# akashsengupta1997/STRAPS-3DHumanShapePose

Measured on AMD Instinct MI355X. Metric: bodies/sec, higher is better.
Workload: dtype fp32 (encoder convolutions as exact bf16x3 operand splits (six bf16 products per term); in-step SMPL blend contraction and skinning as 3-product fp16 splits (fp16x3_lbs: 22-bit operands); fp32 accumulate throughout)

## Files before the change

include/straps_hip.h:

```cpp
#ifndef STRAPS_HIP_H
#define STRAPS_HIP_H

#include <stddef.h>
#include <stdint.h>

#ifdef __cplusplus
extern "C" {
#endif

#define STRAPS_ABI_VERSION 12

#define STRAPS_OK 0
#define STRAPS_EINVAL 1
#define STRAPS_EHIP 2
#define STRAPS_EUNSUPPORTED 3

int straps_abi_version(void);
int straps_selftest_mfma_peak(const float* seed512, float* out, int blocks, int iters, void* stream);
int straps_selftest_mfma_bf16(float* out, unsigned long long* clk2, int blocks, int iters, void* stream);
int straps_selftest_mfma_bf16_dense(float* out, unsigned long long* clk2, int blocks, int iters, int data, void* stream);
const char* straps_last_error(void);
int straps_device_count(void);
int straps_wall_clock_khz(void);
int straps_set_clock_accumulator(unsigned long long* acc2);
// ... 221 lines not shown
                          unsigned short* draw_planes, long long plane_stride, void* workspace, long long rows, int c,
                          int accumulate, void* stream);
int straps_bn_bwd_finish_bits_x3(const float* dy, const unsigned* relu_bits, const float* raw, const float* save_mean,
                                 const float* save_invstd, const float* gamma, float* dgamma, float* dbeta, float* draw,
                                 unsigned short* draw_planes, long long plane_stride, const double* partials, int nblk,
                                 void* workspace, long long rows, int c, int accumulate, void* stream);
int straps_conv_dgrad_x3_bits(const unsigned short* dy3, long long dy_plane_stride, const unsigned short* w3_crsk,
                              long long w_plane_stride, const float* addend, float* dx_nhwc, int batch, int h, int w,
                              int cin, int cout, int kh, int kw, int stride, int pad, int tile_cfg,
                              const unsigned* addend_bits, void* stream);
int straps_conv_dgrad_x3_bn_bits(const unsigned short* dy3, long long dy_plane_stride,
                                 const unsigned short* w3_crsk, long long w_plane_stride, const float* addend,
                                 float* dx_nhwc, int batch, int h, int w, int cin, int cout, int kh, int kw,
                                 int stride, int pad, int tile_cfg, const float* bn_raw, const float* bn_out,
                                 const float* bn_mask_scale, const float* bn_mask_shift, const float* bn_mean,
                                 const float* bn_invstd, double* bn_partials, const unsigned* addend_bits,
                                 const unsigned* bn_out_bits, void* stream);
int straps_conv_wgrad_x3_on_planes(int batch, int h, int w, int cin, int cout, int kh, int kw,
                                   int stride, int pad);
int straps_conv_wgrad_x3(const float* x_nhwc, const float* dy_nhwc, const unsigned short* x3,
                         long long x_plane_stride, const unsigned short* dy3, long long dy_plane_stride,
                         float* dw_oihw, void* workspace, int batch, int h, int w, int cin, int cout,
                         int kh, int kw, int stride, int pad, int accumulate, void* stream);


size_t straps_conv_wgrad_workspace_bytes(int batch, int h, int w, int cin, int cout, int kh,
                                         int kw, int stride, int pad);
int straps_conv_wgrad(const float* x_nhwc, const float* dy_nhwc, float* dw_oihw, void* workspace,
                      int batch, int h, int w, int cin, int cout, int kh, int kw, int stride,
                      int pad, int accumulate, void* stream);
#define STRAPS_WG_ROUTE_F32 0
#define STRAPS_WG_ROUTE_PLANES 1
#define STRAPS_WG_ROUTE_F32_1X1 2
#define STRAPS_WG_FAMILY_TAP_F32 0
#define STRAPS_WG_FAMILY_HALO_F32 1
#define STRAPS_WG_FAMILY_TAP_X3 2
#define STRAPS_WG_FAMILY_HALO_X3 3
#define STRAPS_WG_FAMILY_TAP_X3F 4
typedef struct straps_wgrad_plan_t {
    int32_t family;
    int32_t bco, bci;
    int32_t chunk_px;
    int32_t tiles;
    int32_t splits;
    int32_t unit;
    int32_t units;
    int32_t taps;
    int32_t lds_bytes;
    int64_t part_bytes;
} straps_wgrad_plan_t;
int straps_conv_wgrad_plan(int route, int batch, int h, int w, int cin, int cout, int kh, int kw, int stride, int pad,
                           straps_wgrad_plan_t* out);
size_t straps_stem_wgrad_workspace_bytes(int batch, int cin, int h, int w);
int straps_stem_wgrad(const float* x_nchw, const float* dy_nhwc, float* dw_oihw, void* workspace,
                      const uint32_t* nzmask , int batch, int cin,
                      int h, int w, int accumulate, void* stream);
#define STRAPS_STEM_DGRAD_MAX_CIN 64
size_t straps_stem_dgrad_weight_floats(int cin);
int straps_pack_stem_dgrad_weight(const float* w_oihw, float* w_pk, int cin, void* stream);
int straps_stem_dgrad(const float* dy_nhwc, const float* w_pk, float* dx_nchw, int batch, int cin, int h, int w,
                      int accumulate, void* stream);
int straps_bn_bwd_blocks(long long rows, int c);
size_t straps_bn_bwd_workspace_bytes(long long rows, int c);
int straps_bn_bwd(const float* dy, const float* yact, const float* raw, const float* save_mean,
                  const float* save_invstd, const float* gamma, const float* mask_scale,
                  const float* mask_shift, float* dgamma, float* dbeta, float* draw, float* dz_out,
                  void* workspace, long long rows, int c, int accumulate, void* stream);
int straps_bn_relu_maxpool_fwd(const float* raw_nhwc, const float* scale, const float* shift,
                               float* y_pool_nhwc, uint8_t* idx, int batch, int h, int w, int c,
                               void* stream);
int straps_bn_bwd_pooled(const float* dy_pool_nhwc, const uint8_t* idx, const float* raw,
                         const float* save_mean, const float* save_invstd, const float* gamma,
                         const float* mask_scale, const float* mask_shift, float* dgamma, float* dbeta,
                         float* draw, void* workspace, int batch, int h, int w, int c, int accumulate,
                         void* stream);
size_t straps_stem_tiles(int batch, int in_h, int in_w);
int straps_stem_tile_activity(const uint32_t* nzmask, uint8_t* tile_active, int batch, int cin, int in_h,
                              int in_w, void* stream);
int straps_bn_bwd_pooled_sparse(const float* dy_pool_nhwc, const uint8_t* idx, const float* raw,
                                const float* save_mean, const float* save_invstd, const float* gamma,
                                const float* mask_scale, const float* mask_shift, float* dgamma,
                                float* dbeta, float* draw, void* workspace, int batch, int h, int w, int c,
                                int accumulate, const uint8_t* tile_active, void* stream);
int straps_maxpool_fwd_idx(const float* x_nhwc, float* y_nhwc, uint8_t* idx, int batch, int h,
                           int w, int c, void* stream);
int straps_maxpool_bwd(const float* dy_nhwc, const uint8_t* idx, float* dx_nhwc, int batch, int h,
                       int w, int c, void* stream);
int straps_gap_bwd(const float* dfeat, float* dx_nhwc, int batch, int hw, int c, void* stream);
int straps_masked_copy(const float* x, int ldx, const float* mask, int ldmask, float* y, int ldy,
                       int m, int n, int accumulate, void* stream);
int straps_rot6d_bwd(const float* x6, long long ld, int per_row, const float* drot, float* dx6,
                     long long ldd, long long rows, void* stream);

int straps_build_proxy_input(const float* seg, const float* joints2d, float* out_nchw, int batch,
                             int nj, int wh, void* stream);
int straps_build_proxy_input_std(const float* seg, const float* joints2d, float* out_nchw, int batch,
                                 int nj, int wh, int std, void* stream);
int straps_build_proxy_input_nz(const float* seg, const float* joints2d, float* out_nchw, uint32_t* nzmask,
                                int batch, int nj, int wh, int std, void* stream);
size_t straps_loss_workspace_bytes(long long batch);
int straps_loss_fwd_bwd(const float* pred_verts, const float* pred_joints, const float* est,
                        int ld_est, const float* pred_rot, const float* tgt_verts,
                        const float* tgt_joints2d, const float* tgt_joints3d,
                        const float* tgt_shape, const float* tgt_rot, const float* log_vars,
                        float* loss_out, float* dverts, float* djoints, float* dest, float* drot,
                        float* dlogvar, void* workspace, long long batch, int img_wh, void* stream);
int straps_loss_fwd_bwd_gm(const float* pred_verts, const float* pred_joints, const float* est, int ld_est,
                           const float* pred_rot, const float* tgt_verts, const float* tgt_joints2d,
                           const float* tgt_joints3d, const float* tgt_shape, const float* tgt_rot,
                           const float* log_vars, float* loss_out, float* dverts, float* djoints, float* dest,
                           float* drot, float* dlogvar, void* workspace, long long batch, int img_wh,
                           const float* j2d_count_global, float count_scale, void* stream);
int straps_count_visible(const float* tgt_joints2d, float* out_count, long long batch, int nj, int img_wh,
                         void* stream);
int straps_mse_fwd(const float* pred, const float* tgt, const uint8_t* row_mask, long long rows,
                   int cols, float tgt_scale, float tgt_shift, float* out3, void* workspace,
                   void* stream);
int straps_mse_bwd(const float* pred, const float* tgt, const uint8_t* row_mask, long long rows,
                   int cols, float tgt_scale, float tgt_shift, const float* coef, float* grad,
                   void* stream);
int straps_augment_seg(const float* seg, const float* uniforms, const float* remove_prob,
                       float occlude_prob, int box_dim, float* out, int batch, int wh, void* stream);
int straps_philox_fill(unsigned long long seed, const long long* step_dev, long long step_host,
                       unsigned substream, float* out, long long n, int kind, void* stream);
int straps_counter_add(long long* counters, int n, long long delta, void* stream);
int straps_gather_f32(const float* src, const int* index, float* dst, int n, void* stream);
int straps_memset_zero(void* ptr, size_t bytes, void* stream);
int straps_augment_smpl(const float* pose_rows, long long n_rows, const float* u_index,
                        const float* orig_shape, const float* mean_shape, const float* shape_draws,
                        int shape_mode, const float* std_vector, double range_lo, double range_hi,
                        float* out_shape, float* out_rotmats, float* out_pose, long long batch,
                        void* stream);
int straps_augment_cam_t(const float* mean_cam_t, const float* normals_xy, const float* uniform_z,
                         double xy_std, double z_lo, double z_hi, float* out_cam_t, long long batch,
                         void* stream);
int straps_deviate_joints2d(const float* joints2d, const float* uniforms, double lo, double hi,
                            double hip_lo, double hip_hi, float* out, long long batch, void* stream);
int straps_deviate_verts2d(const float* verts, const float* uniforms, double lo, double hi, float* out,
                           long long nverts_total, void* stream);
int straps_project_targets(const float* joints, const float* cam_t, float fx, float fy, float cx,
                           float cy, float* joints2d, float* joints3d, long long batch, void* stream);
size_t straps_rasterize_workspace_bytes(long long batch, int nverts, int wh);
int straps_rasterize_parts(const float* verts, const int32_t* faces, const uint8_t* face_parts,
                           const float* cam_K, const float* cam_R, const float* cam_t, float* parts,
                           float* depth, void* workspace, long long batch, int nverts, int nfaces, int wh,
                           int cam_per_body, float near, float far, const float* vert_noise_u, double noise_lo,
                           double noise_hi, void* stream);
int straps_crop_resize(const float* seg, const float* joints2d, const float* uniforms,
                       double orig_scale_factor, double delta_scale_lo, double delta_scale_hi,
                       double delta_centre_lo, double delta_centre_hi, float* out_seg,
                       float* out_joints2d, int* boxes, int batch, int wh, int out_wh, int nj,
                       void* stream);
int straps_predict_proxy_input(const uint8_t* sil, const float* joints2d, int ld_joint,
                               const float* gauss_patch, int std, double bbox_scale_factor,
                               float* out_nchw, float* out_joints2d, int32_t* boxes,
                               int batch, int h, int w, int nj, int out_wh, void* stream);
int straps_point_metrics(const float* pred, const float* target, float* out3, long long batch,
                         int npoints, void* stream);
int straps_point_align(const float* pred, const float* target, float* out3, float* pred_sc,
                       float* pred_pa, long long batch, int npoints, void* stream);
int straps_silhouette_counts(const uint8_t* pred, const uint8_t* target, int32_t* counts4,
                             long long batch, long long npix, void* stream);
size_t straps_wp_silhouette_workspace_bytes(long long batch, int nverts);
int straps_wp_silhouette(const float* verts, const int32_t* faces, const float* cam_wp, uint8_t* mask,
                         void* workspace, long long batch, int nverts, int nfaces, int wh, void* stream);
int straps_adam_step(float* params, const float* grads, float* exp_avg, float* exp_avg_sq,
// ... 105 lines not shown
```

straps-3dhumanshapepose_amd/autograd_ops.py:

```python
import ctypes as C

import torch

from . import hipabi
from .encoder_exec import encoder_forward
from .ief_module import EST_LD


def _empty_like(t):
    return torch.empty_like(t, memory_format=torch.contiguous_format)


class GradSink(dict):

    def __init__(self, views=None):
        super().__init__()
        self.views = views

    def buf(self, p, zero=False):
        if self.views is not None and p in self.views:
            return self.views[p]
        return torch.zeros_like(p) if zero else torch.empty_like(p)


# ... 156 lines not shown
                                                   k, k, stride, pad, 0, hipabi.ptr(bn_next['raw']), hipabi.ptr(None if from_raw else bn_next['out']),
                                                   hipabi.ptr(ssn[0] if from_raw else None), hipabi.ptr(ssn[1] if from_raw else None),
                                                   hipabi.ptr(ssn[2]), hipabi.ptr(ssn[3]), hipabi.ptr(part), hipabi.stream_ptr()),
                         'straps_conv_dgrad_x3_bn')
            bn_next['bwd_partials'] = (part, nblk, dx)
            return dx
        if addend_bits is not None:
            hipabi.check(L.straps_conv_dgrad_x3_bits(hipabi.ptr(g3), gps, hipabi.ptr(w3), wps, hipabi.ptr(addend), hipabi.ptr(dx), B, H, W, Cin, Cout,
                                                     k, k, stride, pad, 0, hipabi.ptr(addend_bits), hipabi.stream_ptr()), 'straps_conv_dgrad_x3_bits')
            return dx
        hipabi.check(L.straps_conv_dgrad_x3(hipabi.ptr(g3), gps, hipabi.ptr(w3), wps, hipabi.ptr(addend), hipabi.ptr(dx), B, H, W, Cin, Cout,
                                            k, k, stride, pad, 0, hipabi.stream_ptr()), 'straps_conv_dgrad_x3')
        return dx
    if addend_bits is not None:
        raise RuntimeError('ReLU bits exist only on the bf16x3 route')
    hipabi.check(L.straps_conv_dgrad(hipabi.ptr(draw), hipabi.ptr(_packed_dgrad_weight(net, conv)), hipabi.ptr(addend), hipabi.ptr(dx), B, H, W,
                                     Cin, Cout, k, k, stride, pad, 0, hipabi.stream_ptr()), 'straps_conv_dgrad')
    return dx


def encoder_backward(net, tape, dfeat, views=None, side_stream=None, after_layer3=None, want_dx=False, param_grads=True):
    L = hipabi.lib()
    grads = GradSink(views)
    side = _SideStream(side_stream)
    sink = {} if getattr(net, 'conv_precision', 'fp32') == 'bf16x3' else None

    def sink_of(rec):
        return None if rec.get('fmode') else sink

    def keep(rec):
        if sink is None or rec.get('x3') is None:
            return True
        B, H, W, Cin, Cout, k, stride, pad, Ho, Wo = rec['geom']
        return not L.straps_conv_wgrad_x3_on_planes(B, H, W, Cin, Cout, k, k, stride, pad)
    rec = tape['gap']
    B, HW, Cf = rec['geom']
    dy = _empty_like(rec['x'])
    hipabi.check(L.straps_gap_bwd(hipabi.ptr(dfeat.contiguous()), hipabi.ptr(dy), B, HW, Cf, hipabi.stream_ptr()), 'straps_gap_bwd')
    units = [u for li in range(1, 5) for u in getattr(net, 'layer%d' % li)]
    for li in range(4, 0, -1):
        for unit in reversed(list(getattr(net, 'layer%d' % li))):
            pairs = unit.conv_bn_pairs()
            ui = units.index(unit)
            prev_last = tape[id(units[ui - 1].conv_bn_pairs()[-1][0])] if ui > 0 else None
            rec = tape[id(pairs[-1][0])]
            ubits = rec.get('bits') if sink is not None else None
            dskip_bits = None
            if ubits is not None:
                draw, _ = _bn_bwd(L, rec, dy, True, False, grads, sink_of(rec), keep(rec))
                dz = dy
            else:
                draw, dz = _bn_bwd(L, rec, dy, True, True, grads, sink_of(rec), keep(rec))
            if param_grads:
                side.run(lambda rec=rec, draw=draw: _conv_wgrad(L, rec, draw, grads, sink), draw)
            if unit.downsample is not None:
                recd = tape[id(unit.downsample[0])]
                drawd, _ = _bn_bwd(L, recd, dz, False, False, grads, sink_of(recd), keep(recd), mask_bits=ubits)
                if param_grads:
                    side.run(lambda recd=recd, drawd=drawd: _conv_wgrad(L, recd, drawd, grads, sink), drawd)
                dskip = _conv_dgrad(L, net, recd, drawd, None, sink)
            else:
                dskip, dskip_bits = dz, ubits
            for ci in range(len(pairs) - 1, 0, -1):
                rec_prev = tape[id(pairs[ci - 1][0])]
                dt = _conv_dgrad(L, net, tape[id(pairs[ci][0])], draw, None, sink, bn_next=rec_prev if sink is not None else None)
                rec = rec_prev
                draw, _ = _bn_bwd(L, rec, dt, True, False, grads, sink_of(rec), keep(rec))
                if param_grads:
                    side.run(lambda rec=rec, draw=draw: _conv_wgrad(L, rec, draw, grads, sink), draw)
            dy = _conv_dgrad(L, net, tape[id(pairs[0][0])], draw, dskip, sink, bn_next=prev_last if sink is not None else None,
                             addend_bits=dskip_bits)
        if li == 3 and after_layer3 is not None:
            side.join()
            after_layer3()
    rec = tape['maxpool']
    B, H, W, Cc, Hp, Wp = rec['geom']
    if rec['kind'] == 'maxpool_fused':
        idx = rec['idx']
        rec = tape['stem']
        bn, raw, ss = rec['bn'], rec['raw'], rec['stats']
        ws = torch.empty(L.straps_bn_bwd_workspace_bytes(B * H * W, Cc) // 4, device=raw.device, dtype=torch.float32)
        dgamma, dbeta = grads.buf(bn.weight), grads.buf(bn.bias)
        draw = _empty_like(raw)
        tact = None
        if rec.get('nzmask') is not None and _SPARSE_STEM_TAIL and not want_dx:
            _, Cin0, Hin, Win = rec['geom'][:4]
            tact = torch.empty(L.straps_stem_tiles(B, Hin, Win), device=raw.device, dtype=torch.uint8)
            hipabi.check(L.straps_stem_tile_activity(hipabi.ptr(rec['nzmask']), hipabi.ptr(tact), B, Cin0, Hin, Win, hipabi.stream_ptr()),
                         'straps_stem_tile_activity')
        hipabi.check(L.straps_bn_bwd_pooled_sparse(hipabi.ptr(dy), hipabi.ptr(idx), hipabi.ptr(raw), hipabi.ptr(ss[2]), hipabi.ptr(ss[3]),
                                                   hipabi.ptr(bn.weight), hipabi.ptr(ss[0]), hipabi.ptr(ss[1]), hipabi.ptr(dgamma), hipabi.ptr(dbeta),
                                                   hipabi.ptr(draw), hipabi.ptr(ws), B, H, W, Cc, 2 if rec.get('frozen') else 0, hipabi.ptr(tact),
                                                   hipabi.stream_ptr()), 'straps_bn_bwd_pooled_sparse')
        grads[bn.weight] = dgamma
        grads[bn.bias] = dbeta
    else:
        dstem = _empty_like(rec['x'])
        hipabi.check(L.straps_maxpool_bwd(hipabi.ptr(dy), hipabi.ptr(rec['idx']), hipabi.ptr(dstem), B, H, W, Cc, hipabi.stream_ptr()),
                     'straps_maxpool_bwd')
        rec = tape['stem']
        draw, _ = _bn_bwd(L, rec, dstem, True, False, grads)
    B, Cin, H, W, Ho, Wo = rec['geom']
    dx = None
    if want_dx:
        dx = torch.empty(B, Cin, H, W, device=draw.device, dtype=torch.float32)
        hipabi.check(L.straps_stem_dgrad(hipabi.ptr(draw), hipabi.ptr(net._packed_stem_dgrad_weight()), hipabi.ptr(dx), B, Cin, H, W, 0,
                                         hipabi.stream_ptr()), 'straps_stem_dgrad')
    if param_grads:
        ws = torch.empty(L.straps_stem_wgrad_workspace_bytes(B, Cin, H, W) // 4, device=draw.device, dtype=torch.float32)
        dw = grads.buf(net.conv1.weight)
        hipabi.check(L.straps_stem_wgrad(hipabi.ptr(rec['x']), hipabi.ptr(draw), hipabi.ptr(dw), hipabi.ptr(ws), hipabi.ptr(rec.get('nzmask')),
                                         B, Cin, H, W, 0, hipabi.stream_ptr()), 'straps_stem_wgrad')
        grads[net.conv1.weight] = dw
    side.join()
    return (grads, dx) if want_dx else grads


def ief_backward(ief, feat, tape, dest, views=None, param_grads=True):
    sink = GradSink(views)
    L, st = hipabi.lib(), hipabi.stream_ptr()
    pk = ief._packed(feat.device)
    B, F = feat.shape
    H1, H2, P = ief.fc1.out_features, ief.fc2.out_features, ief.num_output_params
    dev = feat.device
    T = len(tape)
    e = lambda *s: torch.empty(*s, device=dev, dtype=torch.float32)
    D = hipabi.gemm_desc
    ests, h1s, h2s = tape[0]['stacks']
    assert ests.shape == (T + 1, B, EST_LD) and h1s.shape == (T, B, H1) and h2s.shape == (T, B, H2)
    dW3, db3 = sink.buf(ief.fc3.weight), sink.buf(ief.fc3.bias)
    dW2, db2 = sink.buf(ief.fc2.weight), sink.buf(ief.fc2.bias)
    dW1, db1 = sink.buf(ief.fc1.weight), sink.buf(ief.fc1.bias)
    dests = e(T + 1, B, EST_LD)
    dsrc = dest if dest.stride(-1) == 1 and dest.dim() == 2 else dest.contiguous()
    hipabi.check(L.straps_masked_copy(hipabi.ptr(dsrc), dsrc.stride(0), None, 0, hipabi.ptr(dests[T]), EST_LD, B, EST_LD, 0, st), 'ief dest slot')
    dh2s, dh1s, dc1 = e(T, B, H2), e(T, B, H1), e(B, H1)
    w3, w2 = ief.fc3.weight, ief.fc2.weight
    for it in reversed(range(T)):
        hipabi.gemm_multi([D(dests[it + 1], EST_LD, 1, w3, H2, 1, dh2s[it], H2, B, H2, P, mask=h2s[it], ldmask=H2)])
        hipabi.gemm_multi([D(dh2s[it], H2, 1, w2, H1, 1, dh1s[it], H1, B, H1, H2, mask=h1s[it], ldmask=H1,
                             c2=dc1, ldc2=H1, accumulate2=int(it != T - 1))])
        hipabi.gemm_multi([D(dh1s[it], H1, 1, pk['w1e'], EST_LD, 1, dests[it], EST_LD, B, P, H1, addend=dests[it + 1], ldadd=EST_LD)])
    one = pk['one']
    dfeat = e(B, F)
    if not param_grads:
        hipabi.gemm_multi([D(dc1, H1, 1, pk['w1f'], F, 1, dfeat, F, B, F, H1)])
        return dfeat, {}
    KB = T * B
    hipabi.gemm_multi([
        D(dh2s, 1, H2, h1s, H1, 1, dW2, H1, H2, H1, KB),
        D(dc1, 1, H1, feat, F, 1, dW1, F + P, H1, F, B),
        D(dh1s, 1, H1, ests, EST_LD, 1, dW1.data_ptr() + 4 * F, F + P, H1, P, KB),
        D(dests[1], 1, EST_LD, h2s, H2, 1, dW3, H2, P, H2, KB),
        D(dc1, H1, 1, pk['w1f'], F, 1, dfeat, F, B, F, H1),
        D(one, 0, 0, dh2s, H2, 1, db2, H2, 1, H2, KB),
        D(one, 0, 0, dests[1], EST_LD, 1, db3, P, 1, P, KB),
        D(one, 0, 0, dc1, H1, 1, db1, H1, 1, H1, B)])
    grads = {ief.fc1.weight: dW1, ief.fc1.bias: db1, ief.fc2.weight: dW2, ief.fc2.bias: db2, ief.fc3.weight: dW3, ief.fc3.bias: db3}
    return dfeat, grads


class _RegressorFn(torch.autograd.Function):

    @staticmethod
    def forward(ctx, reg, x, *params):
        enc_tape, ief_tape = {}, []
        with torch.no_grad():
            feat = encoder_forward(reg.image_encoder, x, enc_tape)
            est = reg.ief_module.forward_estimate(feat, ief_tape)
        ctx.reg, ctx.feat, ctx.enc_tape, ctx.ief_tape, ctx.params = reg, feat, enc_tape, ief_tape, params
        return est

# ... 171 lines not shown
```

straps-3dhumanshapepose_amd/csrc/backward.hip:

```cpp
#include "common.h"
#include <stdlib.h>

namespace {


constexpr int TY = 2, TX = 32, PH = 2 * TY + 5, PW = 72, TPIX = TY * TX;
constexpr int CG = 4, GK = CG * 49, GNB = (GK + 31) / 32, GUNITS = 2 * GNB, UPW = (GUNITS + 3) / 4;

__global__ __launch_bounds__(256) void stem_tileact_kernel(const unsigned* __restrict__ nzmask, uint8_t* __restrict__ tact, int C, int H, int W,
                                                           int tiles_x, int tiles_y, int ntiles, int groups) {
    const int idx = blockIdx.x * 256 + threadIdx.x;
    if (idx >= ntiles * groups) return;
    const int grp = idx / ntiles, tile = idx - grp * ntiles;
    int bid = tile;
    const int b = bid / (tiles_x * tiles_y);
    bid -= b * tiles_x * tiles_y;
    const int ty = bid / tiles_x, tx = bid - ty * tiles_x;
    const int hi0 = 2 * (ty * TY) - 3, wi0 = 2 * (tx * TX) - 3;
    const int HC = (H + 3) >> 2, WW = (W + 255) >> 8;
    const int rc0 = max(hi0, 0) >> 2, rc1 = min(hi0 + PH - 1, H - 1) >> 2;
    const int wa = max(wi0 - 1, 0), wb = min(wi0 - 2 + PW, W - 1);
    const int c0 = grp * CG, nc = min(CG, C - c0);
    unsigned chact = 0;
    for (int cl = 0; cl < nc; ++cl) {
// ... 343 lines not shown
        double t[8];
#pragma unroll
        for (int e = 0; e < 8; ++e) t[e] = red[tc][e];
        for (int q = 1; q < TR; ++q)
#pragma unroll
            for (int e = 0; e < 8; ++e) t[e] += red[q * 16 + tc][e];
        double* o = part + ((long long)blockIdx.x * C + c4 * 4) * 2;
#pragma unroll
        for (int e = 0; e < 4; ++e) { o[e * 2 + 0] = t[e]; o[e * 2 + 1] = t[4 + e]; }
    }
}

__global__ __launch_bounds__(256) void bn_bwd_reduce_pooled_kernel(const float* __restrict__ raw, const float* __restrict__ mean,
                                                                   const float* __restrict__ invstd, const float* __restrict__ msc,
                                                                   const float* __restrict__ msh, double* __restrict__ part, long long prows,
                                                                   int C, int rows_per_block, PoolSrc ps) {
    __shared__ double red[256][8];
    constexpr int TR = 16;
    const int tc = threadIdx.x & 15, tr = threadIdx.x >> 4;
    const int c4 = blockIdx.y * 16 + tc;
    const bool active = c4 * 4 < C;
    const long long r0 = (long long)blockIdx.x * rows_per_block;
    const long long r1 = r0 + rows_per_block < prows ? r0 + rows_per_block : prows;
    double s1[4] = {0.0, 0.0, 0.0, 0.0}, s2[4] = {0.0, 0.0, 0.0, 0.0};
    f32x4 is = {0.f, 0.f, 0.f, 0.f};
    if (active) {
        const f32x4 mu = *reinterpret_cast<const f32x4*>(mean + c4 * 4);
        is = *reinterpret_cast<const f32x4*>(invstd + c4 * 4);
        const f32x4 ksc = *reinterpret_cast<const f32x4*>(msc + c4 * 4), ksh = *reinterpret_cast<const f32x4*>(msh + c4 * 4);
        for (long long r = r0 + tr; r < r1; r += TR) {
            const int wo = (int)(r % ps.Wo);
            const long long t = r / ps.Wo;
            const int ho = (int)(t % ps.Ho);
            const long long b = t / ps.Ho;
            const long long o = r * C + c4 * 4;
            const f32x4 d = *reinterpret_cast<const f32x4*>(ps.dyp + o);
            const uchar4 k4 = *reinterpret_cast<const uchar4*>(ps.idx + o);
            const int k[4] = {k4.x, k4.y, k4.z, k4.w};
            float xr[4];
#pragma unroll
            for (int e = 0; e < 4; ++e) {
                const int hi = 2 * ho - 1 + k[e] / 3, wi = 2 * wo - 1 + k[e] % 3;
                xr[e] = raw[((b * ps.H + hi) * ps.W + wi) * C + c4 * 4 + e];
            }
#pragma unroll
            for (int e = 0; e < 4; ++e) {
                const float g = fmaf(xr[e], ksc[e], ksh[e]) > 0.f ? d[e] : 0.f;
                s1[e] += (double)g;
                s2[e] += (double)g * ((double)xr[e] - (double)mu[e]);
            }
        }
    }
#pragma unroll
    for (int e = 0; e < 4; ++e) { red[threadIdx.x][e] = s1[e]; red[threadIdx.x][4 + e] = s2[e] * (double)is[e]; }
    __syncthreads();
    if (tr == 0 && active) {
        double t[8];
#pragma unroll
        for (int e = 0; e < 8; ++e) t[e] = red[tc][e];
        for (int q = 1; q < TR; ++q)
#pragma unroll
            for (int e = 0; e < 8; ++e) t[e] += red[q * 16 + tc][e];
        double* o = part + ((long long)blockIdx.x * C + c4 * 4) * 2;
#pragma unroll
        for (int e = 0; e < 4; ++e) { o[e * 2 + 0] = t[e]; o[e * 2 + 1] = t[4 + e]; }
    }
}

__global__ __launch_bounds__(256) void bn_bwd_finalize_kernel(const double* __restrict__ part, int nblocks, int C, double count,
                                                             const float* __restrict__ gamma, const float* __restrict__ invstd,
                                                             float* __restrict__ dgamma, float* __restrict__ dbeta,
                                                             double* __restrict__ coefd, float* __restrict__ k1, int accumulate) {
    int c;
    double s1, s2;
    if (bn_partials_sum4(part, nblocks, C, s1, s2, c)) {
        dbeta[c] = accumulate ? dbeta[c] + (float)s1 : (float)s1;
        dgamma[c] = accumulate ? dgamma[c] + (float)s2 : (float)s2;
        k1[c] = gamma[c] * invstd[c];
        coefd[c] = s1 / count;
        coefd[C + c] = s2 / count;
    }
}

constexpr int POOL_CHUNK = 1024;
template <bool POOL>
__global__ __launch_bounds__(256) void bn_bwd_apply_kernel(const float* __restrict__ dy, const float* __restrict__ yact,
                                                           const float* __restrict__ raw, const float* __restrict__ mean,
                                                           const float* __restrict__ invstd, const double* __restrict__ coefd,
                                                           const float* __restrict__ k1p, const float* __restrict__ msc,
                                                           const float* __restrict__ msh, float* __restrict__ draw, float* dz_out,
                                                           u16* __restrict__ planes, long long pstride, long long n4, int C, PoolSrc ps,
                                                           const unsigned* __restrict__ bits, int tiled) {
    const int C4 = C >> 2;
    const long long first = POOL ? (long long)blockIdx.x * POOL_CHUNK + threadIdx.x : (long long)blockIdx.x * 256 + threadIdx.x;
    const long long last = POOL ? (n4 < ((long long)blockIdx.x + 1) * POOL_CHUNK ? n4 : ((long long)blockIdx.x + 1) * POOL_CHUNK) : n4;
    const long long step = POOL ? 256 : (long long)gridDim.x * 256;
    const long long rows = n4 / C4;
    struct Consts { f32x4 ksc, ksh, mu, is, k1; double m1[4], m2[4]; };
    auto load_consts = [&](int c4) {
        Consts k;
        if (!yact && !bits && msc) { k.ksc = *reinterpret_cast<const f32x4*>(msc + c4 * 4); k.ksh = *reinterpret_cast<const f32x4*>(msh + c4 * 4); }
        k.mu = *reinterpret_cast<const f32x4*>(mean + c4 * 4);
        k.is = *reinterpret_cast<const f32x4*>(invstd + c4 * 4);
        k.k1 = *reinterpret_cast<const f32x4*>(k1p + c4 * 4);
#pragma unroll
        for (int e = 0; e < 4; ++e) { k.m1[e] = coefd[c4 * 4 + e]; k.m2[e] = coefd[C + c4 * 4 + e]; }
        return k;
    };
    auto body = [&](long long idx, long long row, int c4, const Consts& k) {
        f32x4 g;
        if constexpr (POOL) {
            if (ps.tany) {
                const int wi = (int)(row % ps.W);
                const long long t = row / ps.W;
                const int hi = (int)(t % ps.H);
                const long long b = t / ps.H;
                if (!ps.tany[(b * ps.tiles_y + (hi >> 1)) * ps.tiles_x + (wi >> 5)]) return;
            }
            g = pool_grad(ps, row, c4, C);
        } else {
            g = *reinterpret_cast<const f32x4*>(dy + idx * 4);
        }
        const f32x4 xr = *reinterpret_cast<const f32x4*>(raw + idx * 4);
        if (bits) {
            const unsigned nib = bits[row * (C >> 5) + (c4 >> 3)] >> ((c4 & 7) * 4);
#pragma unroll
            for (int e = 0; e < 4; ++e) g[e] = ((nib >> e) & 1u) ? g[e] : 0.f;
        } else if (yact) {
            const f32x4 ya = *reinterpret_cast<const f32x4*>(yact + idx * 4);
#pragma unroll
            for (int e = 0; e < 4; ++e) g[e] = ya[e] > 0.f ? g[e] : 0.f;
        } else if (msc) {
#pragma unroll
            for (int e = 0; e < 4; ++e) g[e] = fmaf(xr[e], k.ksc[e], k.ksh[e]) > 0.f ? g[e] : 0.f;
        }
        f32x4 o;
#pragma unroll
        for (int e = 0; e < 4; ++e) {
            const double xh = ((double)xr[e] - (double)k.mu[e]) * (double)k.is[e];
            o[e] = (float)((double)k.k1[e] * (((double)g[e] - k.m1[e]) - xh * k.m2[e]));
        }
        if (dz_out) *reinterpret_cast<f32x4*>(dz_out + idx * 4) = g;
        if (draw) *reinterpret_cast<f32x4*>(draw + idx * 4) = o;
        if (planes) store_planes4_cm(planes, pstride, row, c4 * 4, rows, o);
    };
    if (!POOL && tiled) {
        const int l = threadIdx.x & 63, w = threadIdx.x >> 6, wcg = tiled, ncb = (C4 >> 4) / wcg, trows = 16 / wcg;
        const int c4 = ((int)(blockIdx.x % ncb) * wcg + w % wcg) * 16 + (l >> 5) * 8 + (l & 7);
        const Consts k = load_consts(c4);
        const long long rstep = (long long)(gridDim.x / ncb) * trows;
        for (long long row = (long long)(blockIdx.x / ncb) * trows + (w / wcg) * 4 + ((l >> 3) & 3); row < rows; row += rstep) body(row * C4 + c4, row, c4, k);
    } else if (step % C4 == 0) {
        if (first >= last) return;
        const int c4 = (int)(first % C4);
        const Consts k = load_consts(c4);
        const long long rstep = step / C4;
        long long row = first / C4;
        for (long long idx = first; idx < last; idx += step, row += rstep) body(idx, row, c4, k);
    } else {
        for (long long idx = first; idx < last; idx += step) {
            const int c4 = (int)(idx % C4);
            body(idx, idx / C4, c4, load_consts(c4));
        }
    }
}

__global__ __launch_bounds__(256) void maxpool_idx_kernel(const float* __restrict__ x, float* __restrict__ y, uint8_t* __restrict__ idx,
                                                          int B, int H, int W, int C, int Ho, int Wo) {
    const int C4 = C >> 2;
    const long long n = (long long)B * Ho * Wo * C4;
    for (long long i = (long long)blockIdx.x * 256 + threadIdx.x; i < n; i += (long long)gridDim.x * 256) {
        const int c4 = (int)(i % C4);
        long long t = i / C4;
        const int wo = (int)(t % Wo); t /= Wo;
        const int ho = (int)(t % Ho);
        const int b = (int)(t / Ho);
        f32x4 m = {-INFINITY, -INFINITY, -INFINITY, -INFINITY};
        int am[4] = {0, 0, 0, 0};
        bool first = true;
#pragma unroll
        for (int r = 0; r < 3; ++r) {
            const int hi = 2 * ho - 1 + r;
            if ((unsigned)hi >= (unsigned)H) continue;
#pragma unroll
            for (int s = 0; s < 3; ++s) {
                const int wi = 2 * wo - 1 + s;
                if ((unsigned)wi >= (unsigned)W) continue;
                const f32x4 v = *reinterpret_cast<const f32x4*>(x + (((long long)b * H + hi) * W + wi) * C + c4 * 4);
#pragma unroll
                for (int e = 0; e < 4; ++e)
                    if (first || v[e] > m[e] || v[e] != v[e]) { m[e] = v[e]; am[e] = r * 3 + s; }
                first = false;
            }
        }
        *reinterpret_cast<f32x4*>(y + i * 4) = m;
        *reinterpret_cast<uchar4*>(idx + i * 4) = make_uchar4((unsigned char)am[0], (unsigned char)am[1], (unsigned char)am[2], (unsigned char)am[3]);
    }
}

__global__ __launch_bounds__(256) void bn_relu_maxpool_kernel(const float* __restrict__ raw, const float* __restrict__ scale,
                                                              const float* __restrict__ shift, float* __restrict__ y, uint8_t* __restrict__ idx,
                                                              u16* __restrict__ planes, long long pstride, int B, int H, int W, int C, int Ho, int Wo) {
    const int C4 = C >> 2;
    const long long n = (long long)B * Ho * Wo * C4;
    for (long long i = (long long)blockIdx.x * 256 + threadIdx.x; i < n; i += (long long)gridDim.x * 256) {
        const int c4 = (int)(i % C4);
        long long t = i / C4;
        const int wo = (int)(t % Wo); t /= Wo;
        const int ho = (int)(t % Ho);
        const int b = (int)(t / Ho);
        const f32x4 sc = *reinterpret_cast<const f32x4*>(scale + c4 * 4);
        const f32x4 sh = *reinterpret_cast<const f32x4*>(shift + c4 * 4);
        f32x4 m = {-INFINITY, -INFINITY, -INFINITY, -INFINITY};
        int am[4] = {0, 0, 0, 0};
        bool first = true;
#pragma unroll
        for (int r = 0; r < 3; ++r) {
            const int hi = 2 * ho - 1 + r;
            if ((unsigned)hi >= (unsigned)H) continue;
#pragma unroll
            for (int s = 0; s < 3; ++s) {
                const int wi = 2 * wo - 1 + s;
                if ((unsigned)wi >= (unsigned)W) continue;
                f32x4 v = *reinterpret_cast<const f32x4*>(raw + (((long long)b * H + hi) * W + wi) * C + c4 * 4);
#pragma unroll
                for (int e = 0; e < 4; ++e) {
                    v[e] = fmaxf(fmaf(v[e], sc[e], sh[e]), 0.f);
                    if (first || v[e] > m[e] || v[e] != v[e]) { m[e] = v[e]; am[e] = r * 3 + s; }
                }
                first = false;
            }
        }
        *reinterpret_cast<f32x4*>(y + i * 4) = m;
        *reinterpret_cast<uchar4*>(idx + i * 4) = make_uchar4((unsigned char)am[0], (unsigned char)am[1], (unsigned char)am[2], (unsigned char)am[3]);
        if (planes) store_planes4_cm(planes, pstride, i / C4, c4 * 4, (long long)B * Ho * Wo, m);
    }
}

__global__ __launch_bounds__(256) void maxpool_bwd_kernel(const float* __restrict__ dy, const uint8_t* __restrict__ idx,
                                                          float* __restrict__ dx, int B, int H, int W, int C, int Ho, int Wo) {
    const int C4 = C >> 2;
    const long long n = (long long)B * H * W * C4;
    for (long long i = (long long)blockIdx.x * 256 + threadIdx.x; i < n; i += (long long)gridDim.x * 256) {
        const int c4 = (int)(i % C4);
        long long t = i / C4;
        const int wi = (int)(t % W); t /= W;
        const int hi = (int)(t % H);
        const int b = (int)(t / H);
        f32x4 g = {0.f, 0.f, 0.f, 0.f};
        const int ho_lo = hi >> 1, ho_hi = (hi + 1) >> 1;
        const int wo_lo = wi >> 1, wo_hi = (wi + 1) >> 1;
        for (int ho = ho_lo; ho <= ho_hi; ++ho) {
            if (ho >= Ho) continue;
            const int r = hi - (2 * ho - 1);
            for (int wo = wo_lo; wo <= wo_hi; ++wo) {
                if (wo >= Wo) continue;
                const int s = wi - (2 * wo - 1);
                const long long o = (((long long)b * Ho + ho) * Wo + wo) * C + c4 * 4;
                const uchar4 k = *reinterpret_cast<const uchar4*>(idx + o);
                const f32x4 d = *reinterpret_cast<const f32x4*>(dy + o);
                const int want = r * 3 + s;
                if (k.x == want) g[0] += d[0];
                if (k.y == want) g[1] += d[1];
                if (k.z == want) g[2] += d[2];
                if (k.w == want) g[3] += d[3];
            }
        }
        *reinterpret_cast<f32x4*>(dx + i * 4) = g;
    }
}

__global__ __launch_bounds__(256) void gap_bwd_kernel(const float* __restrict__ dfeat, float* __restrict__ dx, int B, int HW, int C) {
    const long long n = (long long)B * HW * C;
    const float inv = 1.0f / (float)HW;
    for (long long i = (long long)blockIdx.x * 256 + threadIdx.x; i < n; i += (long long)gridDim.x * 256) {
        const int c = (int)(i % C);
        const long long b = i / ((long long)HW * C);
        dx[i] = dfeat[b * C + c] * inv;
    }
}

__global__ __launch_bounds__(256) void masked_copy_kernel(const float* __restrict__ x, int ldx, const float* __restrict__ mask, int ldm,
                                                          float* y, int ldy, int M, int N, int accumulate) {
    const long long i = (long long)blockIdx.x * 256 + threadIdx.x;
    if (i >= (long long)M * N) return;
    const int m = (int)(i / N), n = (int)(i - (long long)m * N);
    float v = x[(long long)m * ldx + n];
    if (mask) v = mask[(long long)m * ldm + n] > 0.f ? v : 0.f;
    float* o = y + (long long)m * ldy + n;
    *o = accumulate ? *o + v : v;
}

__global__ __launch_bounds__(256) void rot6d_bwd_kernel(const float* __restrict__ x6, long long ld, int per_row,
                                                        const float* __restrict__ dR, float* __restrict__ dx6, long long ldd,
                                                        long long n) {
    const long long idx = (long long)blockIdx.x * 256 + threadIdx.x;
    if (idx >= n) return;
    const long long row = idx / per_row;
    const int j = (int)(idx - row * per_row);
    const float* x = x6 + row * ld + j * 6;
    const float a1[3] = {x[0], x[2], x[4]}, a2[3] = {x[1], x[3], x[5]};
    const float* g = dR + idx * 9;
    float gb1[3] = {g[0], g[3], g[6]}, gb2[3] = {g[1], g[4], g[7]};
    const float gb3[3] = {g[2], g[5], g[8]};
    const float n1r = sqrtf(a1[0] * a1[0] + a1[1] * a1[1] + a1[2] * a1[2]);
    const float n1 = fmaxf(n1r, 1e-12f);
    const float b1[3] = {a1[0] / n1, a1[1] / n1, a1[2] / n1};
    const float d = b1[0] * a2[0] + b1[1] * a2[1] + b1[2] * a2[2];
    const float u[3] = {a2[0] - d * b1[0], a2[1] - d * b1[1], a2[2] - d * b1[2]};
    const float n2r = sqrtf(u[0] * u[0] + u[1] * u[1] + u[2] * u[2]);
    const float n2 = fmaxf(n2r, 1e-12f);
    const float b2[3] = {u[0] / n2, u[1] / n2, u[2] / n2};
    gb1[0] += b2[1] * gb3[2] - b2[2] * gb3[1];
    gb1[1] += b2[2] * gb3[0] - b2[0] * gb3[2];
    gb1[2] += b2[0] * gb3[1] - b2[1] * gb3[0];
    gb2[0] += gb3[1] * b1[2] - gb3[2] * b1[1];
    gb2[1] += gb3[2] * b1[0] - gb3[0] * b1[2];
    gb2[2] += gb3[0] * b1[1] - gb3[1] * b1[0];
// ... 31 lines not shown
}

}

static int stem_wgrad_blocks(int ntiles) {
    static const int cap = STRAPS_TOOL_ENV_INT("STRAPS_STEM_WGRAD_BLOCKS", 256);
    return ntiles < cap ? ntiles : cap;
}

extern "C" size_t straps_stem_wgrad_workspace_bytes(int batch, int cin, int h, int w) {
    const int Ho = (h - 1) / 2 + 1, Wo = (w - 1) / 2 + 1;
    const int ntiles = batch * ((Ho + TY - 1) / TY) * ((Wo + TX - 1) / TX);
    const int Kp = (cin * 49 + 31) / 32 * 32;
    const size_t groups = (cin + CG - 1) / CG;
    return (size_t)stem_wgrad_blocks(ntiles) * 64 * Kp * sizeof(float) + straps_stem_nzmask_words(batch, cin, h, w) * sizeof(uint32_t) +
           ((groups * ntiles + 3) & ~(size_t)3);
}

extern "C" int straps_stem_wgrad(const float* x_nchw, const float* dy_nhwc, float* dw_oihw, void* workspace, const uint32_t* nzmask,
                                 int batch, int cin, int h, int w, int accumulate, void* stream) {
    STRAPS_REQUIRE(x_nchw && dy_nhwc && dw_oihw && workspace, "straps_stem_wgrad: null pointer");
    STRAPS_REQUIRE(batch > 0 && cin > 0 && h >= 7 && w >= 7, "straps_stem_wgrad: bad shape B=%d C=%d H=%d W=%d", batch, cin, h, w);
    const int K = cin * 49, Kp = (K + 31) / 32 * 32;
    const int Ho = (h - 1) / 2 + 1, Wo = (w - 1) / 2 + 1;
    const int tiles_x = (Wo + TX - 1) / TX, tiles_y = (Ho + TY - 1) / TY;
    const int ntiles = batch * tiles_x * tiles_y;
    const int nblk = stem_wgrad_blocks(ntiles);
    const int groups = (cin + CG - 1) / CG;
    STRAPS_REQUIRE(groups <= 65535, "straps_stem_wgrad: too many input channels (%d)", cin);
    hipStream_t st = (hipStream_t)stream;
    float* part = (float*)workspace;
    uint32_t* own = (uint32_t*)(part + (size_t)nblk * 64 * Kp);
    uint8_t* tact = (uint8_t*)(own + straps_stem_nzmask_words(batch, cin, h, w));
    if (!nzmask) {
        const int rc = straps_stem_nzmask(x_nchw, own, batch, cin, h, w, stream);
        if (rc != STRAPS_OK) return rc;
        nzmask = own;
    }
    hipLaunchKernelGGL(stem_tileact_kernel, dim3((ntiles * groups + 255) / 256), dim3(256), 0, st, nzmask, tact, cin, h, w, tiles_x, tiles_y, ntiles,
                       groups);
    STRAPS_CHECK_LAUNCH("stem_tileact_kernel");
    static const int rot = STRAPS_TOOL_ENV_INT("STRAPS_STEM_WGRAD_ROT", 97);
    hipLaunchKernelGGL(stem_wgrad_kernel, dim3(nblk, groups), dim3(256), 0, st, x_nchw, dy_nhwc, part, tact, batch, cin, h, w, Ho, Wo,
                       tiles_x, tiles_y, Kp, ntiles, rot);
    STRAPS_CHECK_LAUNCH("stem_wgrad_kernel");
    hipLaunchKernelGGL(stem_wgrad_reduce_kernel, dim3((64 * K + 63) / 64), dim3(256), 0, st, (const float*)workspace, dw_oihw, nblk, K, Kp, accumulate);
    STRAPS_CHECK_LAUNCH("stem_wgrad_reduce_kernel");
    return STRAPS_OK;
}

static double bn_bwd_count(long long rows, int flags) { return (flags & 2) ? (double)INFINITY : (double)rows; }

extern "C" int straps_bn_bwd_blocks(long long rows, int c) {
    const int colblocks = (c + 63) / 64;
    long long b = 2048 / colblocks;
    const long long cap = (rows + 63) / 64;
    if (b > cap) b = cap;
    return (int)(b < 1 ? 1 : b);
}

static int bn_bwd_x3_impl(const float* dy, const float* yact, const unsigned* relu_bits, const float* raw, const float* save_mean, const float* save_invstd,
                          const float* gamma, const float* mask_scale, const float* mask_shift, float* dgamma, float* dbeta, float* draw,
                          float* dz_out, unsigned short* draw_planes, long long plane_stride, void* workspace, long long rows, int c,
                          int accumulate, void* stream) {
    STRAPS_REQUIRE(!relu_bits || (!yact && (c & 31) == 0), "straps_bn_bwd_bits_x3: the bits replace yact (and need c %% 32 == 0; c=%d)", c);
    STRAPS_REQUIRE(!draw_planes || (plane_stride >= rows * c && plane_stride % 8 == 0), "straps_bn_bwd_x3: plane_stride must be >= rows*c and a multiple of 8");
    STRAPS_REQUIRE(!draw_planes || (c & 31) == 0, "straps_bn_bwd_x3: chunk-major planes need c %% 32 == 0 (c=%d)", c);
    STRAPS_REQUIRE(dy && raw && save_mean && save_invstd && gamma && dgamma && dbeta && (draw || draw_planes) && workspace, "straps_bn_bwd: null pointer");
    STRAPS_REQUIRE(rows > 0 && c > 0 && (c & 3) == 0, "straps_bn_bwd: bad shape rows=%lld c=%d", rows, c);
    const int C4 = c >> 2;
    STRAPS_REQUIRE(C4 <= 256 ? (256 % C4 == 0) : (C4 % 256 == 0), "straps_bn_bwd: channel count %d not supported", c);
    hipStream_t st = (hipStream_t)stream;
    const int nblk = straps_bn_bwd_blocks(rows, c);
    const int rpb = (int)((rows + nblk - 1) / nblk);
    double* part = (double*)workspace;
    double* coefd = part + (size_t)nblk * c * 2;
    float* k1 = (float*)(coefd + 2 * (size_t)c);
    hipLaunchKernelGGL(bn_bwd_reduce_kernel<false>, dim3(nblk, (c + 63) / 64), dim3(256), 0, st, dy, yact, raw, save_mean, save_invstd, mask_scale, mask_shift, part, rows, c, rpb, PoolSrc{}, relu_bits);
    STRAPS_CHECK_LAUNCH("bn_bwd_reduce_kernel");
    hipLaunchKernelGGL(bn_bwd_finalize_kernel, dim3((c + 3) / 4), dim3(256), 0, st, part, nblk, c, bn_bwd_count(rows, accumulate), gamma, save_invstd, dgamma, dbeta, coefd, k1, accumulate & 1);
    STRAPS_CHECK_LAUNCH("bn_bwd_finalize_kernel");
    const long long n4 = rows * C4;
    const int tiled = straps_bn_tiled(rows, c >> 2);
    hipLaunchKernelGGL(bn_bwd_apply_kernel<false>, dim3(tiled ? straps_bn_tiled_grid(rows, c >> 2, tiled) : straps_grid256_rows(n4, c >> 2)), dim3(256), 0, st, dy, yact, raw, save_mean, save_invstd, coefd, k1, mask_scale, mask_shift, draw, dz_out, draw_planes, plane_stride, n4, c, PoolSrc{}, relu_bits, tiled);
    STRAPS_CHECK_LAUNCH("bn_bwd_apply_kernel");
    return STRAPS_OK;
}

extern "C" int straps_bn_bwd_x3(const float* dy, const float* yact, const float* raw, const float* save_mean, const float* save_invstd,
                                const float* gamma, const float* mask_scale, const float* mask_shift, float* dgamma, float* dbeta, float* draw,
                                float* dz_out, unsigned short* draw_planes, long long plane_stride, void* workspace, long long rows, int c,
                                int accumulate, void* stream) {
    return bn_bwd_x3_impl(dy, yact, nullptr, raw, save_mean, save_invstd, gamma, mask_scale, mask_shift, dgamma, dbeta, draw, dz_out, draw_planes,
                          plane_stride, workspace, rows, c, accumulate, stream);
}

extern "C" int straps_bn_bwd_bits_x3(const float* dy, const unsigned* relu_bits, const float* raw, const float* save_mean, const float* save_invstd,
                                     const float* gamma, float* dgamma, float* dbeta, float* draw, unsigned short* draw_planes, long long plane_stride,
                                     void* workspace, long long rows, int c, int accumulate, void* stream) {
    STRAPS_REQUIRE(relu_bits, "straps_bn_bwd_bits_x3: null bit mask");
    return bn_bwd_x3_impl(dy, nullptr, relu_bits, raw, save_mean, save_invstd, gamma, nullptr, nullptr, dgamma, dbeta, draw, nullptr, draw_planes,
                          plane_stride, workspace, rows, c, accumulate, stream);
}

static int bn_bwd_finish_x3_impl(const float* dy, const float* yact, const unsigned* relu_bits, const float* raw, const float* save_mean,
                                 const float* save_invstd, const float* gamma, const float* mask_scale, const float* mask_shift, float* dgamma,
                                 float* dbeta, float* draw, float* dz_out, unsigned short* draw_planes, long long plane_stride, const double* partials,
                                 int nblk, void* workspace, long long rows, int c, int accumulate, void* stream) {
    STRAPS_REQUIRE(!relu_bits || (!yact && (c & 31) == 0), "straps_bn_bwd_finish_bits_x3: the bits replace yact (and need c %% 32 == 0; c=%d)", c);
    STRAPS_REQUIRE(!draw_planes || (plane_stride >= rows * c && plane_stride % 8 == 0), "straps_bn_bwd_finish_x3: plane_stride must be >= rows*c and a multiple of 8");
    STRAPS_REQUIRE(!draw_planes || (c & 31) == 0, "straps_bn_bwd_finish_x3: chunk-major planes need c %% 32 == 0 (c=%d)", c);
    STRAPS_REQUIRE(dy && raw && save_mean && save_invstd && gamma && dgamma && dbeta && (draw || draw_planes) && workspace && partials && nblk > 0,
                   "straps_bn_bwd_finish_x3: null pointer");
    STRAPS_REQUIRE(rows > 0 && c > 0 && (c & 3) == 0, "straps_bn_bwd_finish_x3: bad shape rows=%lld c=%d", rows, c);
    const int C4 = c >> 2;
    STRAPS_REQUIRE(C4 <= 256 ? (256 % C4 == 0) : (C4 % 256 == 0), "straps_bn_bwd_finish_x3: channel count %d not supported", c);
    hipStream_t st = (hipStream_t)stream;
    double* coefd = (double*)workspace;
    float* k1 = (float*)(coefd + 2 * (size_t)c);
    hipLaunchKernelGGL(bn_bwd_finalize_kernel, dim3((c + 3) / 4), dim3(256), 0, st, partials, nblk, c, bn_bwd_count(rows, accumulate), gamma, save_invstd, dgamma, dbeta, coefd, k1, accumulate & 1);
    STRAPS_CHECK_LAUNCH("bn_bwd_finalize_kernel");
    const long long n4 = rows * C4;
    const int tiled = straps_bn_tiled(rows, c >> 2);
    hipLaunchKernelGGL(bn_bwd_apply_kernel<false>, dim3(tiled ? straps_bn_tiled_grid(rows, c >> 2, tiled) : straps_grid256_rows(n4, c >> 2)), dim3(256), 0, st, dy, yact, raw, save_mean, save_invstd, coefd, k1, mask_scale, mask_shift, draw, dz_out, draw_planes, plane_stride, n4, c, PoolSrc{}, relu_bits, tiled);
    STRAPS_CHECK_LAUNCH("bn_bwd_apply_kernel");
    return STRAPS_OK;
}

extern "C" int straps_bn_bwd_finish_x3(const float* dy, const float* yact, const float* raw, const float* save_mean, const float* save_invstd,
                                       const float* gamma, const float* mask_scale, const float* mask_shift, float* dgamma, float* dbeta,
                                       float* draw, float* dz_out, unsigned short* draw_planes, long long plane_stride, const double* partials,
                                       int nblk, void* workspace, long long rows, int c, int accumulate, void* stream) {
    return bn_bwd_finish_x3_impl(dy, yact, nullptr, raw, save_mean, save_invstd, gamma, mask_scale, mask_shift, dgamma, dbeta, draw, dz_out, draw_planes,
                                 plane_stride, partials, nblk, workspace, rows, c, accumulate, stream);
}

extern "C" int straps_bn_bwd_finish_bits_x3(const float* dy, const unsigned* relu_bits, const float* raw, const float* save_mean,
                                            const float* save_invstd, const float* gamma, float* dgamma, float* dbeta, float* draw,
                                            unsigned short* draw_planes, long long plane_stride, const double* partials, int nblk, void* workspace,
                                            long long rows, int c, int accumulate, void* stream) {
    STRAPS_REQUIRE(relu_bits, "straps_bn_bwd_finish_bits_x3: null bit mask");
    return bn_bwd_finish_x3_impl(dy, nullptr, relu_bits, raw, save_mean, save_invstd, gamma, nullptr, nullptr, dgamma, dbeta, draw, nullptr, draw_planes,
                                 plane_stride, partials, nblk, workspace, rows, c, accumulate, stream);
}

extern "C" int straps_bn_bwd(const float* dy, const float* yact, const float* raw, const float* save_mean, const float* save_invstd,
                             const float* gamma, const float* mask_scale, const float* mask_shift, float* dgamma, float* dbeta, float* draw,
                             float* dz_out, void* workspace, long long rows, int c, int accumulate, void* stream) {
    return straps_bn_bwd_x3(dy, yact, raw, save_mean, save_invstd, gamma, mask_scale, mask_shift, dgamma, dbeta, draw, dz_out, nullptr, 0, workspace,
                            rows, c, accumulate, stream);
}

extern "C" size_t straps_stem_tiles(int batch, int h, int w) {
    const int Ho = (h - 1) / 2 + 1, Wo = (w - 1) / 2 + 1;
    return (size_t)batch * ((Wo + TX - 1) / TX) * ((Ho + TY - 1) / TY);
}

extern "C" int straps_stem_tile_activity(const uint32_t* nzmask, uint8_t* tile_active, int batch, int cin, int h, int w, void* stream) {
    STRAPS_REQUIRE(nzmask && tile_active, "straps_stem_tile_activity: null pointer");
    STRAPS_REQUIRE(batch > 0 && cin > 0 && h >= 7 && w >= 7, "straps_stem_tile_activity: bad shape B=%d C=%d H=%d W=%d", batch, cin, h, w);
    const int Ho = (h - 1) / 2 + 1, Wo = (w - 1) / 2 + 1;
    const int tiles_x = (Wo + TX - 1) / TX, tiles_y = (Ho + TY - 1) / TY;
    const int ntiles = batch * tiles_x * tiles_y;
    hipLaunchKernelGGL(stem_tileany_kernel, dim3((unsigned)(((long long)ntiles * 32 + 255) / 256)), dim3(256), 0, (hipStream_t)stream, nzmask, tile_active, cin, h, w, tiles_x, tiles_y,
                       ntiles);
    STRAPS_CHECK_LAUNCH("stem_tileany_kernel");
    return STRAPS_OK;
}

extern "C" int straps_bn_bwd_pooled(const float* dy_pool, const uint8_t* idx, const float* raw, const float* save_mean, const float* save_invstd,
                                    const float* gamma, const float* mask_scale, const float* mask_shift, float* dgamma, float* dbeta,
                                    float* draw, void* workspace, int batch, int h, int w, int c, int accumulate, void* stream) {
    return straps_bn_bwd_pooled_sparse(dy_pool, idx, raw, save_mean, save_invstd, gamma, mask_scale, mask_shift, dgamma, dbeta, draw, workspace, batch, h, w,
                                       c, accumulate, nullptr, stream);
}

extern "C" int straps_bn_bwd_pooled_sparse(const float* dy_pool, const uint8_t* idx, const float* raw, const float* save_mean, const float* save_invstd,
                                           const float* gamma, const float* mask_scale, const float* mask_shift, float* dgamma, float* dbeta,
                                           float* draw, void* workspace, int batch, int h, int w, int c, int accumulate,
                                           const uint8_t* tile_active, void* stream) {
    STRAPS_REQUIRE(dy_pool && idx && raw && save_mean && save_invstd && gamma && mask_scale && mask_shift && dgamma && dbeta && draw && workspace,
                   "straps_bn_bwd_pooled: null pointer");
    STRAPS_REQUIRE(batch > 0 && h > 0 && w > 0 && c > 0 && (c & 3) == 0, "straps_bn_bwd_pooled: bad shape %dx%dx%dx%d", batch, h, w, c);
    const int C4 = c >> 2;
    STRAPS_REQUIRE(C4 <= 256 ? (256 % C4 == 0) : (C4 % 256 == 0), "straps_bn_bwd_pooled: channel count %d not supported", c);
    hipStream_t st = (hipStream_t)stream;
    const long long rows = (long long)batch * h * w;
    const int nblk = straps_bn_bwd_blocks(rows, c);
    const int rpb = (int)((rows + nblk - 1) / nblk);
    double* part = (double*)workspace;
    double* coefd = part + (size_t)nblk * c * 2;
    float* k1 = (float*)(coefd + 2 * (size_t)c);
    const PoolSrc ps{dy_pool, idx, h, w, (h - 1) / 2 + 1, (w - 1) / 2 + 1, tile_active, (w + TX - 1) / TX, (h + TY - 1) / TY};
    const long long prows = (long long)batch * ps.Ho * ps.Wo;
    const int prpb = (int)((prows + nblk - 1) / nblk);
    (void)rpb;
    hipLaunchKernelGGL(bn_bwd_reduce_pooled_kernel, dim3(nblk, (c + 63) / 64), dim3(256), 0, st, raw, save_mean, save_invstd, mask_scale, mask_shift, part, prows, c, prpb, ps);
    STRAPS_CHECK_LAUNCH("bn_bwd_reduce_pooled_kernel");
    hipLaunchKernelGGL(bn_bwd_finalize_kernel, dim3((c + 3) / 4), dim3(256), 0, st, part, nblk, c, bn_bwd_count(rows, accumulate), gamma, save_invstd, dgamma, dbeta, coefd, k1, accumulate & 1);
    STRAPS_CHECK_LAUNCH("bn_bwd_finalize_kernel");
    const long long n4 = rows * C4;
    hipLaunchKernelGGL(bn_bwd_apply_kernel<true>, dim3((unsigned)((n4 + POOL_CHUNK - 1) / POOL_CHUNK)), dim3(256), 0, st, nullptr, nullptr, raw, save_mean, save_invstd, coefd, k1, mask_scale, mask_shift, draw, nullptr, (u16*)nullptr, 0LL, n4, c, ps, (const unsigned*)nullptr, 0);
    STRAPS_CHECK_LAUNCH("bn_bwd_apply_kernel<pool>");
    return STRAPS_OK;
}

extern "C" int straps_bn_relu_maxpool_fwd_x3(const float* raw, const float* scale, const float* shift, float* y_pool, uint8_t* idx,
                                             unsigned short* y_planes, long long plane_stride, int batch, int h, int w, int c, void* stream) {
    STRAPS_REQUIRE(raw && scale && shift && y_pool && idx && batch > 0 && h > 0 && w > 0 && c > 0 && (c & 3) == 0, "straps_bn_relu_maxpool_fwd: bad arguments");
    const int Ho = (h - 1) / 2 + 1, Wo = (w - 1) / 2 + 1;
    const long long n = (long long)batch * Ho * Wo * (c >> 2);
    STRAPS_REQUIRE(!y_planes || (plane_stride >= n * 4 && plane_stride % 8 == 0), "straps_bn_relu_maxpool_fwd_x3: plane_stride must be >= the output size and a multiple of 8");
    STRAPS_REQUIRE(!y_planes || (c & 31) == 0, "straps_bn_relu_maxpool_fwd_x3: chunk-major planes need c %% 32 == 0 (c=%d)", c);
    hipLaunchKernelGGL(bn_relu_maxpool_kernel, dim3(capped_grid(n)), dim3(256), 0, (hipStream_t)stream, raw, scale, shift, y_pool, idx, y_planes, plane_stride, batch, h, w, c, Ho, Wo);
    STRAPS_CHECK_LAUNCH("bn_relu_maxpool_kernel");
    return STRAPS_OK;
}

extern "C" int straps_bn_relu_maxpool_fwd(const float* raw, const float* scale, const float* shift, float* y_pool, uint8_t* idx, int batch, int h,
                                          int w, int c, void* stream) {
    return straps_bn_relu_maxpool_fwd_x3(raw, scale, shift, y_pool, idx, nullptr, 0, batch, h, w, c, stream);
}

extern "C" size_t straps_bn_bwd_workspace_bytes(long long rows, int c) {
    return ((size_t)straps_bn_bwd_blocks(rows, c) * c * 2 + 2 * (size_t)c) * sizeof(double) + (size_t)c * sizeof(float);
}

extern "C" int straps_maxpool_fwd_idx(const float* x, float* y, uint8_t* idx, int batch, int h, int w, int c, void* stream) {
    STRAPS_REQUIRE(x && y && idx, "straps_maxpool_fwd_idx: null pointer");
    STRAPS_REQUIRE(batch > 0, "straps_maxpool_fwd_idx: batch must be positive (batch=%d)", batch);
    STRAPS_REQUIRE(h > 0, "straps_maxpool_fwd_idx: h must be positive (h=%d)", h);
    STRAPS_REQUIRE(w > 0, "straps_maxpool_fwd_idx: w must be positive (w=%d)", w);
    STRAPS_REQUIRE(c > 0 && (c & 3) == 0, "straps_maxpool_fwd_idx: c must be a positive multiple of 4 (c=%d)", c);
    const int Ho = (h - 1) / 2 + 1, Wo = (w - 1) / 2 + 1;
    const long long n = (long long)batch * Ho * Wo * (c >> 2);
    hipLaunchKernelGGL(maxpool_idx_kernel, dim3(capped_grid(n)), dim3(256), 0, (hipStream_t)stream, x, y, idx, batch, h, w, c, Ho, Wo);
    STRAPS_CHECK_LAUNCH("maxpool_idx_kernel");
    return STRAPS_OK;
}

extern "C" int straps_maxpool_bwd(const float* dy, const uint8_t* idx, float* dx, int batch, int h, int w, int c, void* stream) {
    STRAPS_REQUIRE(dy && idx && dx, "straps_maxpool_bwd: null pointer");
    STRAPS_REQUIRE(batch > 0, "straps_maxpool_bwd: batch must be positive (batch=%d)", batch);
    STRAPS_REQUIRE(h > 0, "straps_maxpool_bwd: h must be positive (h=%d)", h);
    STRAPS_REQUIRE(w > 0, "straps_maxpool_bwd: w must be positive (w=%d)", w);
    STRAPS_REQUIRE(c > 0 && (c & 3) == 0, "straps_maxpool_bwd: c must be a positive multiple of 4 (c=%d)", c);
    const int Ho = (h - 1) / 2 + 1, Wo = (w - 1) / 2 + 1;
    const long long n = (long long)batch * h * w * (c >> 2);
    hipLaunchKernelGGL(maxpool_bwd_kernel, dim3(capped_grid(n)), dim3(256), 0, (hipStream_t)stream, dy, idx, dx, batch, h, w, c, Ho, Wo);
    STRAPS_CHECK_LAUNCH("maxpool_bwd_kernel");
    return STRAPS_OK;
}

extern "C" int straps_gap_bwd(const float* dfeat, float* dx, int batch, int hw, int c, void* stream) {
    STRAPS_REQUIRE(dfeat && dx && batch > 0 && hw > 0 && c > 0, "straps_gap_bwd: bad arguments");
    const long long n = (long long)batch * hw * c;
    hipLaunchKernelGGL(gap_bwd_kernel, dim3(capped_grid(n)), dim3(256), 0, (hipStream_t)stream, dfeat, dx, batch, hw, c);
    STRAPS_CHECK_LAUNCH("gap_bwd_kernel");
    return STRAPS_OK;
}

extern "C" int straps_masked_copy(const float* x, int ldx, const float* mask, int ldmask, float* y, int ldy, int m, int n, int accumulate,
                                  void* stream) {
    STRAPS_REQUIRE(x && y && m > 0 && n > 0, "straps_masked_copy: bad arguments");
    const long long t = (long long)m * n;
    hipLaunchKernelGGL(masked_copy_kernel, dim3((unsigned)((t + 255) / 256)), dim3(256), 0, (hipStream_t)stream, x, ldx, mask, ldmask, y, ldy, m, n, accumulate);
    STRAPS_CHECK_LAUNCH("masked_copy_kernel");
    return STRAPS_OK;
}

extern "C" int straps_rot6d_bwd(const float* x6, long long ld, int per_row, const float* drot, float* dx6, long long ldd, long long rows,
                                void* stream) {
    STRAPS_REQUIRE(x6 && drot && dx6 && rows > 0 && per_row > 0, "straps_rot6d_bwd: bad arguments");
    const long long n = rows * per_row;
    hipLaunchKernelGGL(rot6d_bwd_kernel, dim3((unsigned)((n + 255) / 256)), dim3(256), 0, (hipStream_t)stream, x6, ld, per_row, drot, dx6, ldd, n);
    STRAPS_CHECK_LAUNCH("rot6d_bwd_kernel");
    return STRAPS_OK;
}
```

straps-3dhumanshapepose_amd/csrc/regressor_train.hip:

```cpp
#include <algorithm>
#include <cstring>

#include "regressor_net.h"

namespace {

constexpr long long kX3fMinRows = 16384;
constexpr size_t kNone = ~(size_t)0;

struct Layer : Conv, Extent {
    long long rows;
    bool fmode;
    bool keep, planes, defer, bits;
    bool keep_grad;
    int nblk;
    size_t x, x3;
    long long x_ps;
    const Layer* a_bn;
    size_t raw, ss, out, out3, bitsb;
    long long out_ps;
};

struct Plan : Net {
    bool x3;
// ... 191 lines not shown
    STRAPS_REQUIRE(params, "%s: null pointer `params`", fn);
    STRAPS_REQUIRE(((uintptr_t)params & 15) == 0, "%s: `params` must be 16-byte aligned", fn);
    make_net(d, p);
    STRAPS_REQUIRE(make_plan(p, batch, h, w), "%s: input %d x %d is too small for resnet%d", fn, h, w, p.layers);
    return STRAPS_OK;
}

int finalize(const float* params, float* bn_state, const float* part, int nblk, int c, long long rows, long long gb, long long rs, float* ss,
             hipStream_t st) {
    return straps_bn_stats_finalize(part, nblk, c, rows, params + gb, params + gb + c, kBnEps, kBnMomentum, bn_state + rs, bn_state + rs + c,
                                    ss, ss + c, ss + 2 * c, ss + 3 * c, st);
}

}

extern "C" size_t straps_regressor_train_param_floats(const straps_regressor_desc_t* d) {
    if (check_desc(d, true)) return 0;
    Net n;
    make_net(d, n);
    return (size_t)n.train_floats;
}

extern "C" size_t straps_regressor_bn_state_floats(const straps_regressor_desc_t* d) {
    if (check_desc(d, true)) return 0;
    Net n;
    make_net(d, n);
    return (size_t)n.bn_floats;
}

extern "C" size_t straps_regressor_train_workspace_bytes(const straps_regressor_desc_t* d, int batch, int h, int w) {
    if (check_desc(d, true)) return 0;
    Plan p;
    make_net(d, p);
    if (!make_plan(p, batch, h, w)) return 0;
    return p.bytes;
}

extern "C" int straps_regressor_fwd_train(const straps_regressor_desc_t* d, const float* params, float* bn_state, const float* init_est,
                                          const float* x, int batch, int h, int w, float* est, int ld_est, void* workspace,
                                          size_t workspace_bytes, void* stream) {
    static const char* fn = "straps_regressor_fwd_train";
    Plan p;
    RG_CALL(check_common(fn, d, params, x, batch, h, w, workspace, p));
    STRAPS_REQUIRE(bn_state, "%s: null pointer `bn_state`", fn);
    STRAPS_REQUIRE(init_est, "%s: null pointer `init_est`", fn);
    STRAPS_REQUIRE(est, "%s: null pointer `est`", fn);
    STRAPS_REQUIRE(ld_est >= kNumParams, "%s: `ld_est` must be >= %d (got %d)", fn, kNumParams, ld_est);
    STRAPS_REQUIRE(((uintptr_t)bn_state & 3) == 0 && ((uintptr_t)init_est & 3) == 0 && ((uintptr_t)est & 3) == 0,
                   "%s: `bn_state`, `init_est` and `est` must be float-aligned", fn);
    STRAPS_REQUIRE(workspace_bytes >= p.bytes, "%s: `workspace_bytes` is %zu, this batch needs %zu (straps_regressor_train_workspace_bytes)", fn,
                   workspace_bytes, p.bytes);
    hipStream_t st = (hipStream_t)stream;
    const Ws ws{(char*)workspace};
    const int B = batch, C = p.cin, F = p.F, H1 = p.H1, H2 = p.H2;
    const bool x3 = p.x3;
    unsigned short* krsc3 = ws.h(p.krsc);
    float* krsc = ws.f(p.krsc);

    RG_CALL(straps_pack_stem_weight(params + p.stem.w_off, ws.f(p.wstem), C, stream));
    PackTable tbl;
    memset(&tbl, 0, sizeof(tbl));
    for (int i = 0; i < p.nconvs; ++i) {
        const Conv& cv = p.convs[i];
        straps_pack_desc_t& e = tbl.d[i];
        e.src = params + cv.w_off;
        e.dst_krsc = x3 ? nullptr : ws.f(p.krsc) + cv.first;
        e.dst_crsk = x3 ? nullptr : ws.f(p.crsk) + cv.first;
        e.o = cv.cout; e.c = cv.cin; e.r = cv.k; e.s = cv.k;
        e.first = cv.first;
    }
    straps_pack_desc_t* table = (straps_pack_desc_t*)(ws.base + p.table);
    hipLaunchKernelGGL(write_table_kernel, dim3(1), dim3(64), 0, st, tbl, p.nconvs, table, ws.f(p.one));
    STRAPS_CHECK_LAUNCH("write_table_kernel");
    if (x3) RG_CALL(straps_pack_conv_weights_batched_x3(table, p.nconvs, p.conv_total, krsc3, ws.h(p.crsk), p.ps, stream));
    else RG_CALL(straps_pack_conv_weights_batched(table, p.nconvs, p.conv_total, stream));
    RG_CALL(straps_ief_pack(params + p.ief.fc1w, params + p.ief.fc3w, ws.f(p.w1f), ws.f(p.w1e), ws.f(p.w3), F, kNumParams, H1, H2, kEstLd, stream));

    uint32_t* nz = (uint32_t*)(ws.base + p.nz);
    float* part = ws.f(p.fpart);
    float* sss = ws.f(p.stem_ss);
    RG_CALL(straps_stem_nzmask(x, nz, B, C, h, w, stream));
    RG_CALL(straps_stem_fwd(x, ws.f(p.wstem), nullptr, nullptr, 0, ws.f(p.stem_raw), part, nz, B, C, h, w, stream));
    RG_CALL(finalize(params, bn_state, part, p.stem_nblk, 64, (long long)B * p.geo.Hs * p.geo.Ws, p.stem.gb_off, p.stem.rs_off, sss, st));
    if (p.pool_planes)
        RG_CALL(straps_bn_relu_maxpool_fwd_x3(ws.f(p.stem_raw), sss, sss + 64, ws.f(p.pool), (uint8_t*)(ws.base + p.idx), ws.h(p.pool3), p.pool_ps,
                                              B, p.geo.Hs, p.geo.Ws, 64, stream));
    else
        RG_CALL(straps_bn_relu_maxpool_fwd(ws.f(p.stem_raw), sss, sss + 64, ws.f(p.pool), (uint8_t*)(ws.base + p.idx), B, p.geo.Hs, p.geo.Ws, 64, stream));

    auto conv_fwd = [&](const Layer& cv) -> int {
        const float* sa = cv.a_bn ? ws.f(cv.a_bn->ss) : nullptr;
        if (cv.fmode)
            return straps_conv_fwd_x3f(ws.f(cv.x), sa, sa ? sa + cv.a_bn->cout : nullptr, cv.a_bn ? 1 : 0, krsc3 + cv.first, p.ps, nullptr, nullptr,
                                       nullptr, 0, ws.f(cv.raw), part, B, cv.H, cv.W, cv.cin, cv.cout, cv.k, cv.k, cv.stride, cv.pad, 0, stream);
        if (x3)
            return straps_conv_fwd_x3(ws.h(cv.x3), cv.x_ps, krsc3 + cv.first, p.ps, nullptr, nullptr, nullptr, 0, ws.f(cv.raw), part,
                                      B, cv.H, cv.W, cv.cin, cv.cout, cv.k, cv.k, cv.stride, cv.pad, 0, stream);
        return straps_conv_fwd(ws.f(cv.x), krsc + cv.first, nullptr, nullptr, nullptr, 0, ws.f(cv.raw), part, B, cv.H, cv.W, cv.cin, cv.cout,
                               cv.k, cv.k, cv.stride, cv.pad, 0, stream);
    };
    auto conv_bn = [&](const Layer& cv, const float* residual) -> int {
        RG_CALL(conv_fwd(cv));
        float* ss = ws.f(cv.ss);
        RG_CALL(finalize(params, bn_state, part, cv.nblk, cv.cout, cv.rows, cv.gb_off, cv.rs_off, ss, st));
        if (cv.defer) return STRAPS_OK;
        if (x3 && cv.relu) {
            if (cv.bits)
                return straps_bn_apply_bits_x3(ws.f(cv.raw), ss, ss + cv.cout, residual, ws.f(cv.out), ws.h(cv.out3), cv.out_ps, ws.u(cv.bitsb),
                                               cv.rows, cv.cout, stream);
            return straps_bn_apply_x3(ws.f(cv.raw), ss, ss + cv.cout, residual, 1, ws.f(cv.out), ws.h(cv.out3), cv.out_ps, cv.rows, cv.cout, stream);
        }
        return straps_bn_apply(ws.f(cv.raw), ss, ss + cv.cout, residual, cv.relu ? 1 : 0, ws.f(cv.out), cv.rows, cv.cout, stream);
    };
    for (int ui = 0; ui < p.nunits; ++ui) {
        const Unit& u = p.units[ui];
        const float* idt = ws.f(p.lay[u.c[0]].x);
        if (u.has_ds) {
            RG_CALL(conv_bn(p.lay[u.ds], nullptr));
            idt = ws.f(p.lay[u.ds].out);
        }
        for (int ci = 0; ci < u.nconv; ++ci) RG_CALL(conv_bn(p.lay[u.c[ci]], p.lay[u.c[ci]].last ? idt : nullptr));
    }

    RG_CALL(ief_forward(p, B, ws.f(p.unit_out(p.nunits - 1).out), p.geo.Hf * p.geo.Wf, init_est, ws.f(p.w1f), ws.f(p.w1e), params + p.ief.fc1b,
                        params + p.ief.fc2w, params + p.ief.fc2b, ws.f(p.w3), params + p.ief.fc3b, ws.f(p.feat), ws.f(p.c1), ws.f(p.ests),
                        ws.f(p.h1s), (long long)B * H1, ws.f(p.h2s), (long long)B * H2, est, ld_est, stream));
    return STRAPS_OK;
}

extern "C" int straps_regressor_bwd(const straps_regressor_desc_t* d, const float* params, const float* x, int batch, int h, int w,
                                    const float* dest, int ld_dest, float* grads, float* dx, void* workspace, size_t workspace_bytes,
                                    void* stream) {
    static const char* fn = "straps_regressor_bwd";
    Plan p;
    RG_CALL(check_common(fn, d, params, x, batch, h, w, workspace, p));
    STRAPS_REQUIRE(dest, "%s: null pointer `dest`", fn);
    STRAPS_REQUIRE(ld_dest >= kNumParams, "%s: `ld_dest` must be >= %d (got %d)", fn, kNumParams, ld_dest);
    STRAPS_REQUIRE(((uintptr_t)dest & 3) == 0 && ((uintptr_t)grads & 3) == 0 && ((uintptr_t)dx & 3) == 0,
                   "%s: `dest`, `grads` and `dx` must be float-aligned", fn);
    STRAPS_REQUIRE(!dx || p.cin <= STRAPS_STEM_DGRAD_MAX_CIN, "%s: `dx` needs `in_channels` <= %d (got %d)", fn, STRAPS_STEM_DGRAD_MAX_CIN, p.cin);
    STRAPS_REQUIRE(workspace_bytes >= p.bytes, "%s: `workspace_bytes` is %zu, this batch needs %zu (straps_regressor_train_workspace_bytes)", fn,
                   workspace_bytes, p.bytes);
    const Ws ws{(char*)workspace};
    const int B = batch, C = p.cin, F = p.F, H1 = p.H1, H2 = p.H2, T = p.iters, P = kNumParams;
    const bool x3 = p.x3, pg = grads != nullptr;
    const unsigned short* crsk3 = ws.h(p.crsk);
    const float* crsk = ws.f(p.crsk);
    float* dgb = ws.f(p.dgb);
    auto dgamma = [&](long long gb) { return pg ? grads + gb : dgb; };
    auto dbeta = [&](long long gb, int c) { return pg ? grads + gb + c : dgb + 2048; };

    float* dests = ws.f(p.dests);
    float* dh2s = ws.f(p.dh2s);
    float* dh1s = ws.f(p.dh1s);
    float* dc1 = ws.f(p.dc1);
    float* dfeat = ws.f(p.dfeat);
    const float* ests = ws.f(p.ests);
    const float* h1s = ws.f(p.h1s);
    const float* h2s = ws.f(p.h2s);
    RG_CALL(straps_masked_copy(dest, ld_dest, nullptr, 0, dests + (size_t)T * B * kEstLd, kEstLd, B, P, 0, stream));
    auto gd = [](const float* a, long long sam, long long sak, const float* b, long long sbk, long long sbn, float* c, int ldc, int m, int n, int k) {
        straps_gemm_desc_t g;
        memset(&g, 0, sizeof(g));
        g.a = a; g.sam = sam; g.sak = sak; g.b = b; g.sbk = sbk; g.sbn = sbn; g.c = c; g.ldc = ldc; g.m = m; g.n = n; g.k = k;
        return g;
    };
    for (int it = T - 1; it >= 0; --it) {
        float* dnext = dests + (size_t)(it + 1) * B * kEstLd;
        float* dh2 = dh2s + (size_t)it * B * H2;
        float* dh1 = dh1s + (size_t)it * B * H1;
        straps_gemm_desc_t g = gd(dnext, kEstLd, 1, params + p.ief.fc3w, H2, 1, dh2, H2, B, H2, P);
// ... 84 lines not shown
            if (bn_next) {
                const float* ssn = ws.f(bn_next->ss);
                const int cn = bn_next->cout;
                const bool from_raw = !bn_next->last;
                nbits = from_raw ? nullptr : ws.u(bn_next->bitsb);
                if (from_raw || nbits) {
                    nblk = straps_conv_dgrad_x3f_bn_blocks(B, cv.H, cv.W, cv.cin, cv.cout, cv.k, cv.k, cv.stride, cv.pad, 0);
                    prt = part;
                    raw = ws.f(bn_next->raw); mean = ssn + 2 * cn; invstd = ssn + 3 * cn;
                    if (from_raw) { msc = ssn; msh = ssn + cn; }
                }
            }
            RG_CALL(straps_conv_dgrad_x3f(ws.f(draw_off), crsk3 + cv.first, p.ps, addend, addend_bits, out, B, cv.H, cv.W, cv.cin, cv.cout, cv.k, cv.k,
                                          cv.stride, cv.pad, 0, raw, nbits, msc, msh, mean, invstd, prt, stream));
            if (prt) { pending = bn_next; pending_nblk = nblk; }
            return STRAPS_OK;
        }
        if (x3) {
            const unsigned short* g3 = ws.h(draw3_off);
            const unsigned short* w3 = crsk3 + cv.first;
            if (bn_next) {
                const float* ssn = ws.f(bn_next->ss);
                const int cn = bn_next->cout;
                const bool from_raw = !bn_next->last;
                const int nblk = straps_conv_dgrad_x3_bn_blocks(B, cv.H, cv.W, cv.cin, cv.cout, cv.k, cv.k, cv.stride, cv.pad, 0);
                const unsigned* nbits = from_raw ? nullptr : ws.u(bn_next->bitsb);
                if (addend_bits || nbits)
                    RG_CALL(straps_conv_dgrad_x3_bn_bits(g3, gps, w3, p.ps, addend, out, B, cv.H, cv.W, cv.cin, cv.cout, cv.k, cv.k, cv.stride, cv.pad, 0,
                                                         ws.f(bn_next->raw), (from_raw || nbits) ? nullptr : ws.f(bn_next->out),
                                                         from_raw ? ssn : nullptr, from_raw ? ssn + cn : nullptr, ssn + 2 * cn, ssn + 3 * cn, part,
                                                         addend_bits, nbits, stream));
                else
                    RG_CALL(straps_conv_dgrad_x3_bn(g3, gps, w3, p.ps, addend, out, B, cv.H, cv.W, cv.cin, cv.cout, cv.k, cv.k, cv.stride, cv.pad, 0,
                                                    ws.f(bn_next->raw), from_raw ? nullptr : ws.f(bn_next->out), from_raw ? ssn : nullptr,
                                                    from_raw ? ssn + cn : nullptr, ssn + 2 * cn, ssn + 3 * cn, part, stream));
                pending = bn_next;
                pending_nblk = nblk;
                return STRAPS_OK;
            }
            if (addend_bits)
                return straps_conv_dgrad_x3_bits(g3, gps, w3, p.ps, addend, out, B, cv.H, cv.W, cv.cin, cv.cout, cv.k, cv.k, cv.stride, cv.pad, 0,
                                                 addend_bits, stream);
            return straps_conv_dgrad_x3(g3, gps, w3, p.ps, addend, out, B, cv.H, cv.W, cv.cin, cv.cout, cv.k, cv.k, cv.stride, cv.pad, 0, stream);
        }
        return straps_conv_dgrad(ws.f(draw_off), crsk + cv.first, addend, out, B, cv.H, cv.W, cv.cin, cv.cout, cv.k, cv.k, cv.stride, cv.pad, 0, stream);
    };
    for (int ui = p.nunits - 1; ui >= 0; --ui) {
        const Unit& u = p.units[ui];
        const Layer* prev_last = ui > 0 ? &p.unit_out(ui - 1) : nullptr;
        const Layer& lc = p.unit_out(ui);
        const float* dy = ws.f(p.g[cur]);
        const unsigned* ubits = x3 ? ws.u(lc.bitsb) : nullptr;
        const float* dz = dy;
        if (ubits) {
            RG_CALL(bn_bwd(lc, dy, true, nullptr, nullptr, p.draw, p.draw3));
        } else {
            RG_CALL(bn_bwd(lc, dy, true, ws.f(p.dz), nullptr, p.draw, p.draw3));
            dz = ws.f(p.dz);
        }
        RG_CALL(wgrad(lc, p.draw, p.draw3));
        const float* dskip = dz;
        const unsigned* dskip_bits = nullptr;
        if (u.has_ds) {
            const Layer& ds = p.lay[u.ds];
            RG_CALL(bn_bwd(ds, dz, false, nullptr, ubits, p.drawd, p.drawd3));
            RG_CALL(wgrad(ds, p.drawd, p.drawd3));
            RG_CALL(dgrad(ds, p.drawd, p.drawd3, nullptr, nullptr, nullptr, ws.f(p.dskip)));
            dskip = ws.f(p.dskip);
        } else {
            dskip_bits = ubits;
        }
        for (int ci = u.nconv - 1; ci > 0; --ci) {
            const Layer& prev = p.lay[u.c[ci - 1]];
            RG_CALL(dgrad(p.lay[u.c[ci]], p.draw, p.draw3, nullptr, nullptr, x3 ? &prev : nullptr, ws.f(p.dt)));
            RG_CALL(bn_bwd(prev, ws.f(p.dt), true, nullptr, nullptr, p.draw, p.draw3));
            RG_CALL(wgrad(prev, p.draw, p.draw3));
        }
        RG_CALL(dgrad(p.lay[u.c[0]], p.draw, p.draw3, dskip, dskip_bits, x3 ? prev_last : nullptr, ws.f(p.g[cur ^ 1])));
        cur ^= 1;
    }

    const float* sss = ws.f(p.stem_ss);
    const uint32_t* nz = (const uint32_t*)(ws.base + p.nz);
    uint8_t* tact = nullptr;
    if (!dx) {
        tact = (uint8_t*)(ws.base + p.tact);
        RG_CALL(straps_stem_tile_activity(nz, tact, B, C, h, w, stream));
    }
    float* sdraw = ws.f(p.sdraw);
    RG_CALL(straps_bn_bwd_pooled_sparse(ws.f(p.g[cur]), (const uint8_t*)(ws.base + p.idx), ws.f(p.stem_raw), sss + 128, sss + 192, params + p.stem.gb_off,
                                        sss, sss + 64, dgamma(p.stem.gb_off), dbeta(p.stem.gb_off, 64), sdraw, bnws, B, p.geo.Hs, p.geo.Ws, 64, 0, tact, stream));
    if (dx) {
        RG_CALL(straps_pack_stem_dgrad_weight(params + p.stem.w_off, ws.f(p.wsd), C, stream));
        RG_CALL(straps_stem_dgrad(sdraw, ws.f(p.wsd), dx, B, C, h, w, 0, stream));
    }
    if (pg) RG_CALL(straps_stem_wgrad(x, sdraw, grads + p.stem.w_off, ws.base + p.swgws, nz, B, C, h, w, 0, stream));
    return STRAPS_OK;
}

extern "C" int straps_regressor_export_infer_params(const straps_regressor_desc_t* d, const float* params, const float* bn_state,
                                                    const float* init_est, float* infer_params, void* stream) {
    static const char* fn = "straps_regressor_export_infer_params";
    const char* bad = check_desc(d, true);
    STRAPS_REQUIRE(!bad, "%s: %s", fn, bad);
    STRAPS_REQUIRE(params, "%s: null pointer `params`", fn);
    STRAPS_REQUIRE(bn_state, "%s: null pointer `bn_state`", fn);
    STRAPS_REQUIRE(init_est, "%s: null pointer `init_est`", fn);
    STRAPS_REQUIRE(infer_params, "%s: null pointer `infer_params`", fn);
    Net n;
    make_net(d, n);
    hipStream_t st = (hipStream_t)stream;
    auto copy = [&](long long dst, const float* src, long long count) -> int {
        const hipError_t e = hipMemcpyAsync(infer_params + dst, src, (size_t)count * sizeof(float), hipMemcpyDeviceToDevice, st);
        if (e != hipSuccess) {
            straps_set_error("%s: hipMemcpyAsync failed: %s", fn, hipGetErrorString(e));
            return STRAPS_EHIP;
        }
        return STRAPS_OK;
    };
    auto layer = [&](const Conv& cv) -> int {
        RG_CALL(copy(cv.inf_w, params + cv.w_off, cv.weights()));
        RG_CALL(copy(cv.inf_bn, params + cv.gb_off, 2LL * cv.cout));
        return copy(cv.inf_bn + 2LL * cv.cout, bn_state + cv.rs_off, 2LL * cv.cout);
    };
    RG_CALL(layer(n.stem));
    for (int i = 0; i < n.nconvs; ++i) RG_CALL(layer(n.convs[i]));
    RG_CALL(copy(n.ief_inf.fc1w, params + n.ief.fc1w, n.train_floats - n.ief.fc1w));
    RG_CALL(copy(n.inf_init, init_est, kNumParams));
    return STRAPS_OK;
}
```

straps-3dhumanshapepose_amd/encoder_exec.py:

```python
import torch

from . import hipabi


X3F_MIN_ROWS = 16384
X3F_OPERAND_BN = True


def x3f_mode(ctx, conv, B, H, W):
    if not ctx.x3 or not X3F_MIN_ROWS:
        return False
    Cout, Cin, k = conv.weight.shape[0], conv.weight.shape[1], conv.weight.shape[2]
    stride, pad = conv.stride[0], conv.padding[0]
    if not ctx.L.straps_conv_x3f_supported(Cin, Cout, k, conv.weight.shape[3], stride, pad):
        return False
    Ho, Wo = _conv_out(H, k, stride, pad), _conv_out(W, k, stride, pad)
    return B * Ho * Wo >= X3F_MIN_ROWS


_RELU_BITS = True

def _conv_out(h, k, s, p):
    return (h + 2 * p - k) // s + 1

# ... 126 lines not shown
        x1, _ = _planes_of(ctx, x)
        hipabi.check(L.straps_conv_fwd_bf16(hipabi.ptr(x1), hipabi.ptr(net._packed_weight_bf16(conv)), s0, s1, hipabi.ptr(residual), int(relu),
                                            hipabi.ptr(y), None, B, H, W, Cin, Cout, k, k, stride, pad, tile_cfg, hipabi.stream_ptr()),
                     'straps_conv_fwd_bf16')
        return
    if getattr(net, 'conv_precision', 'fp32') == 'bf16x3':
        x3, xps = _planes_of(ctx, x)
        w3, wps = net._packed_weight_x3(conv)
        hipabi.check(L.straps_conv_fwd_x3(hipabi.ptr(x3), xps, hipabi.ptr(w3), wps, s0, s1, hipabi.ptr(residual), int(relu), hipabi.ptr(y),
                                          hipabi.ptr(part), B, H, W, Cin, Cout, k, k, stride, pad, tile_cfg, hipabi.stream_ptr()),
                     'straps_conv_fwd_x3')
    else:
        hipabi.check(L.straps_conv_fwd(hipabi.ptr(x), hipabi.ptr(wpk), s0, s1, hipabi.ptr(residual), int(relu), hipabi.ptr(y),
                                       hipabi.ptr(part), B, H, W, Cin, Cout, k, k, stride, pad, tile_cfg, hipabi.stream_ptr()),
                     'straps_conv_fwd')


def conv_stat_blocks(L, net, geom, Ho, Wo, tile_cfg, fmode=False):
    B, H, W, Cin, Cout, k, stride, pad = geom
    if fmode:
        return L.straps_conv_x3f_stat_blocks(B, H, W, Cin, Cout, k, k, stride, pad, tile_cfg)
    if getattr(net, 'conv_precision', 'fp32') == 'bf16x3':
        return L.straps_conv_x3_stat_blocks(B, H, W, Cin, Cout, k, k, stride, pad, tile_cfg)
    return L.straps_conv_stat_blocks(B, Ho, Wo, Cout, k * k * Cin, tile_cfg)


def conv_bn(ctx, net, x, B, H, W, conv, bn, relu, residual=None, tile_cfg=0, keep_fp32=True, planes=True, a_bn=None, defer_apply=False):
    L = ctx.L
    Cout, Cin, k = conv.weight.shape[0], conv.weight.shape[1], conv.weight.shape[2]
    stride, pad = conv.stride[0], conv.padding[0]
    Ho, Wo = _conv_out(H, k, stride, pad), _conv_out(W, k, stride, pad)
    wpk = None if (ctx.x3 or ctx.bf16) else net._packed_weight(conv)
    y = ctx.empty(B, Ho, Wo, Cout)
    rec = None
    if ctx.tape is not None:
        rec = dict(kind='conv', conv=conv, bn=bn, x=x, geom=(B, H, W, Cin, Cout, k, stride, pad, Ho, Wo), relu=relu,
                   residual=residual)
        ctx.tape[id(conv)] = rec
    if not ctx.training and rec is None:
        ss = net._folded_bn(bn)
        if ctx.x3 and relu:
            x3, xps = _planes_of(ctx, x)
            w3, wps = net._packed_weight_x3(conv)
            if not keep_fp32:
                y = x.new_empty(0)
            yps = (B * Ho * Wo * Cout + 7) // 8 * 8
            yp = torch.empty(3, yps, device=x.device, dtype=torch.int16)
            hipabi.check(L.straps_conv_fwd_x3p(hipabi.ptr(x3), xps, hipabi.ptr(w3), wps, hipabi.ptr(ss[0]), hipabi.ptr(ss[1]), hipabi.ptr(residual), int(relu),
                                               hipabi.ptr(y if keep_fp32 else None), hipabi.ptr(yp), yps, B, H, W, Cin, Cout, k, k, stride, pad, tile_cfg,
                                               hipabi.stream_ptr()), 'straps_conv_fwd_x3p')
            ctx.planes[id(y)] = (y, yp, yps)
            return y, Ho, Wo
        if ctx.bf16 and relu:
            x1, _ = _planes_of(ctx, x)
            if not keep_fp32:
                y = x.new_empty(0)
            yp = torch.empty((B * Ho * Wo * Cout + 7) // 8 * 8, device=x.device, dtype=torch.int16)
            hipabi.check(L.straps_conv_fwd_bf16(hipabi.ptr(x1), hipabi.ptr(net._packed_weight_bf16(conv)), hipabi.ptr(ss[0]), hipabi.ptr(ss[1]),
                                                hipabi.ptr(residual), int(relu), hipabi.ptr(y if keep_fp32 else None), hipabi.ptr(yp), B, H, W, Cin, Cout,
                                                k, k, stride, pad, tile_cfg, hipabi.stream_ptr()), 'straps_conv_fwd_bf16')
            ctx.planes[id(y)] = (y, yp, 0)
            return y, Ho, Wo
        _conv_launch(ctx, net, x, wpk, conv, ss, residual, relu, y, None, (B, H, W, Cin, Cout, k, stride, pad), tile_cfg)
        return y, Ho, Wo
    fmode = rec is not None and x3f_mode(ctx, conv, B, H, W) and x.numel() > 0
    if a_bn is not None and not fmode:
        raise RuntimeError('operand-path BatchNorm needs the fp32-operand route')
    nblk, part = 0, None
    if ctx.training:
        nblk = conv_stat_blocks(L, net, (B, H, W, Cin, Cout, k, stride, pad), Ho, Wo, tile_cfg, fmode)
        part = ctx.empty(nblk, Cout, 2)
    _conv_launch(ctx, net, x, wpk, conv, None, None, False, y, part, (B, H, W, Cin, Cout, k, stride, pad), tile_cfg, fmode, a_bn)
    if rec is not None and ctx.x3:
        rec['x3'] = ctx.planes.get(id(x))
        rec['fmode'] = fmode
        rec['a_bn'] = a_bn
    if defer_apply:
        ss = _bn_train_finish(ctx, bn, y, part, nblk, B * Ho * Wo, None, relu, rec, apply=False)
        return (y, ss), Ho, Wo
    out = _bn_train_finish(ctx, bn, y, part, nblk, B * Ho * Wo, residual, relu, rec, keep_fp32=keep_fp32, planes=planes)
    return out, Ho, Wo


def encoder_forward(net, x, tape=None, nzmask=None):
    hipabi.require_gpu_tensor(x, 'encoder input', torch.float32)
    if x.dim() != 4 or x.shape[1] != net.in_channels:
        raise RuntimeError('encoder expects [B,%d,H,W], got %s' % (net.in_channels, tuple(x.shape)))
    hipabi.require_gpu_tensor(net.conv1.weight, 'encoder parameters (call .to(device))')
    x = x.contiguous()
    B, C, H, W = x.shape
    ctx = _Ctx(x.device, net.training, tape)
    ctx.net = net
    ctx.x3 = getattr(net, 'conv_precision', 'fp32') == 'bf16x3'
    ctx.bf16 = getattr(net, 'conv_precision', 'fp32') == 'bf16'
    if ctx.bf16 and (net.training or tape is not None):
        raise RuntimeError("conv_precision='bf16' is an inference-only route: no train-mode or taped forward (use torch.no_grad() and .eval())")
    if net.training:
        net._bn_epoch = getattr(net, '_bn_epoch', 0) + 1
    ctx.defer_nbt = getattr(net, '_nbt_flat', None) is not None
    L = ctx.L
    Ho, Wo = _conv_out(H, 7, 2, 3), _conv_out(W, 7, 2, 3)
    wfrag = net._packed_weight(net.conv1, stem=True)
    y = ctx.empty(B, Ho, Wo, 64)
    rec = None
    if tape is not None:
        rec = dict(kind='stem', conv=net.conv1, bn=net.bn1, x=x, geom=(B, C, H, W, Ho, Wo), relu=True, residual=None)
        tape["stem"] = rec
    nwords = L.straps_stem_nzmask_words(B, C, H, W)
    if getattr(net, 'dense_stem', False):
        nzmask = torch.empty(nwords, device=x.device, dtype=torch.int32)
        nzmask.fill_(-1)
    elif nzmask is not None:
        if nzmask.dtype != torch.int32 or nzmask.numel() != nwords or nzmask.device != x.device or not nzmask.is_contiguous():
            raise RuntimeError('encoder_forward: nzmask must be a contiguous int32 tensor of %d words on %s' % (nwords, x.device))
    else:
        nzmask = torch.empty(nwords, device=x.device, dtype=torch.int32)
        hipabi.check(L.straps_stem_nzmask(hipabi.ptr(x), hipabi.ptr(nzmask), B, C, H, W, hipabi.stream_ptr()), 'straps_stem_nzmask')
    if rec is not None:
        rec['nzmask'] = nzmask
    if not net.training and tape is None:
        ss = net._folded_bn(net.bn1)
        hipabi.check(L.straps_stem_fwd(hipabi.ptr(x), hipabi.ptr(wfrag), hipabi.ptr(ss[0]), hipabi.ptr(ss[1]), 1, hipabi.ptr(y),
                                       None, hipabi.ptr(nzmask), B, C, H, W, hipabi.stream_ptr()), 'straps_stem_fwd')
    else:
        nblk = L.straps_stem_stat_blocks(B, H, W)
        part = ctx.empty(nblk, 64, 2)
        hipabi.check(L.straps_stem_fwd(hipabi.ptr(x), hipabi.ptr(wfrag), None, None, 0, hipabi.ptr(y), hipabi.ptr(part), hipabi.ptr(nzmask),
                                       B, C, H, W, hipabi.stream_ptr()), 'straps_stem_fwd')
        if tape is not None and not getattr(net, 'unfused_stem_tail', False):
            ss = _bn_train_finish(ctx, net.bn1, y, part, nblk, B * Ho * Wo, None, True, rec, apply=False)
            H, W = Ho, Wo
            Hp, Wp = _conv_out(H, 3, 2, 1), _conv_out(W, 3, 2, 1)
            p = ctx.empty(B, Hp, Wp, 64)
            idx = torch.empty(B, Hp, Wp, 64, device=x.device, dtype=torch.uint8)
            u0 = net.layer1[0]
            cons = [u0.conv_bn_pairs()[0][0]] + ([u0.downsample[0]] if u0.downsample is not None else [])
            if ctx.x3 and not all(x3f_mode(ctx, cv, B, Hp, Wp) for cv in cons):
                planes, pstride = _new_planes(p)
                hipabi.check(L.straps_bn_relu_maxpool_fwd_x3(hipabi.ptr(y), hipabi.ptr(ss[0]), hipabi.ptr(ss[1]), hipabi.ptr(p), hipabi.ptr(idx),
                                                             hipabi.ptr(planes), pstride, B, H, W, 64, hipabi.stream_ptr()),
                             'straps_bn_relu_maxpool_fwd_x3')
                ctx.planes[id(p)] = (p, planes, pstride)
            else:
                hipabi.check(L.straps_bn_relu_maxpool_fwd(hipabi.ptr(y), hipabi.ptr(ss[0]), hipabi.ptr(ss[1]), hipabi.ptr(p), hipabi.ptr(idx),
                                                          B, H, W, 64, hipabi.stream_ptr()), 'straps_bn_relu_maxpool_fwd')
            tape['maxpool'] = dict(kind='maxpool_fused', out=p, idx=idx, geom=(B, H, W, 64, Hp, Wp))
            return _residual_stages(ctx, net, p, B, Hp, Wp, tape)
        y = _bn_train_finish(ctx, net.bn1, y, part, nblk, B * Ho * Wo, None, True, rec, planes=False)
    H, W = Ho, Wo
    Hp, Wp = _conv_out(H, 3, 2, 1), _conv_out(W, 3, 2, 1)
    p = ctx.empty(B, Hp, Wp, 64)
    if tape is not None:
        idx = torch.empty(B, Hp, Wp, 64, device=x.device, dtype=torch.uint8)
        hipabi.check(L.straps_maxpool_fwd_idx(hipabi.ptr(y), hipabi.ptr(p), hipabi.ptr(idx), B, H, W, 64, hipabi.stream_ptr()),
                     'straps_maxpool_fwd_idx')
        tape['maxpool'] = dict(kind='maxpool', x=y, out=p, idx=idx, geom=(B, H, W, 64, Hp, Wp))
    else:
        hipabi.check(L.straps_maxpool_fwd(hipabi.ptr(y), hipabi.ptr(p), B, H, W, 64, hipabi.stream_ptr()), 'straps_maxpool_fwd')
    return _residual_stages(ctx, net, p, B, Hp, Wp, tape)


def _residual_stages(ctx, net, y, B, H, W, tape):
    L = ctx.L
    train_tape = ctx.x3 and tape is not None
    units = [u for li in range(1, 5) for u in getattr(net, 'layer%d' % li)]

    def needs(t_conv, b, h, w):
        if x3f_mode(ctx, t_conv, b, h, w):
            return True, False
        k2, s2, p2 = t_conv.weight.shape[2], t_conv.stride[0], t_conv.padding[0]
        return (not L.straps_conv_wgrad_x3_on_planes(b, h, w, t_conv.weight.shape[1], t_conv.weight.shape[0], k2, k2, s2, p2)), True
    for ui, unit in enumerate(units):
        idt = y
        if unit.downsample is not None:
            idt, _, _ = conv_bn(ctx, net, y, B, H, W, unit.downsample[0], unit.downsample[1], relu=False)
        pairs = unit.conv_bn_pairs()
        t, h, w = y, H, W
        a_bn = None
        for ci, (conv, bn) in enumerate(pairs):
            last = ci == len(pairs) - 1
            keep, planes = True, True
            if (ctx.x3 or ctx.bf16) and not ctx.training and tape is None:
                keep = last
            ho2, wo2 = _conv_out(h, conv.weight.shape[2], conv.stride[0], conv.padding[0]), _conv_out(w, conv.weight.shape[2], conv.stride[0], conv.padding[0])
            defer = False
            if train_tape and not last:
                keep, planes = needs(pairs[ci + 1][0], B, ho2, wo2)
                defer = X3F_OPERAND_BN and keep and not planes
            elif train_tape and last:
                planes = False
                if ui + 1 < len(units):
                    nxt = units[ui + 1]
                    cons = [nxt.conv_bn_pairs()[0][0]] + ([nxt.downsample[0]] if nxt.downsample is not None else [])
                    planes = any(needs(cv, B, ho2, wo2)[1] for cv in cons)
            t, h, w = conv_bn(ctx, net, t, B, h, w, conv, bn, relu=True, residual=idt if last else None, keep_fp32=keep, planes=planes, a_bn=a_bn,
                              defer_apply=defer)
            a_bn = None
            if defer:
                t, a_bn = t
        y, H, W = t, h, w
    Cf = y.shape[3]
    feat = ctx.empty(B, Cf)
    hipabi.check(L.straps_gap_fwd(hipabi.ptr(y), hipabi.ptr(feat), B, H * W, Cf, hipabi.stream_ptr()), 'straps_gap_fwd')
    if tape is not None:
        tape["gap"] = dict(kind="gap", x=y, geom=(B, H * W, Cf))
    return feat
```

straps-3dhumanshapepose_amd/hipabi.py:

```python
import ctypes as C
import os
import subprocess

_HERE = os.path.dirname(os.path.abspath(__file__))
CSRC = os.path.join(_HERE, 'csrc')
LIB_PATH = os.path.join(CSRC, 'libstraps_hip.so')
HEADER = os.path.join(os.path.dirname(_HERE), 'include', 'straps_hip.h')
SOURCES = ['abi.hip', 'augment.hip', 'pose.hip', 'ief.hip', 'elementwise.hip', 'conv.hip', 'conv_x3.hip', 'conv_x3_lean.hip', 'conv_bf16.hip', 'conv_x3f.hip', 'conv_wgrad_x3f.hip', 'stem.hip', 'stem_dgrad.hip', 'smpl.hip',
           'smpl_bwd.hip', 'backward.hip', 'conv_wgrad.hip', 'train.hip', 'metrics.hip', 'image.hip', 'raster.hip', 'exchange.hip',
           'regressor.hip', 'regressor_train.hip', 'predict.hip', 'eval.hip', 'fit.hip', 'silfit.hip', 'render.hip', 'measure.hip']

_lib = None
LINK_LIBS = ['-ldl']
EXTRA_FLAGS = {'smpl.hip': ['-fno-slp-vectorize']}


def _existing_sources():
    return [os.path.join(CSRC, s) for s in SOURCES if os.path.isfile(os.path.join(CSRC, s))]


TOOLS_LIB_PATH = os.path.join(os.path.dirname(_HERE), 'tools', 'bin', 'libstraps_hip_tools.so')


def build(force=False, verbose=False, tools=False):
# ... 139 lines not shown
    'straps_set_clock_accumulator': (_I, [_P]),
    'straps_selftest_mfma_peak': (_I, [_P, _P, _I, _I, _P]),
    'straps_selftest_mfma_bf16': (_I, [_P, _P, _I, _I, _P]),
    'straps_selftest_mfma_bf16_dense': (_I, [_P, _P, _I, _I, _I, _P]),
    'straps_pack_conv_weight': (_I, [_P, _P, _I, _I, _I, _I, _P]),
    'straps_pack_conv_weight_dgrad': (_I, [_P, _P, _I, _I, _I, _I, _P]),
    'straps_pack_conv_weights_batched': (_I, [_P, _I, _L, _P]),
    'straps_pack_conv_weights_batched_x3': (_I, [_P, _I, _L, _P, _P, _L, _P]),
    'straps_stem_weight_floats': (_Z, [_I]),
    'straps_pack_stem_weight': (_I, [_P, _P, _I, _P]),
    'straps_bn_fold': (_I, [_P, _P, _P, _P, _F, _P, _P, _I, _P]),
    'straps_bn_fold_stats': (_I, [_P, _P, _P, _P, _F, _P, _P, _P, _P, _I, _P]),
    'straps_stem_stat_blocks': (_I, [_I, _I, _I]),
    'straps_stem_nzmask_words': (_Z, [_I, _I, _I, _I]),
    'straps_stem_nzmask': (_I, [_P, _P, _I, _I, _I, _I, _P]),
    'straps_stem_fwd': (_I, [_P, _P, _P, _P, _I, _P, _P, _P, _I, _I, _I, _I, _P]),
    'straps_conv_trace_buffer': (_I, [_P]),
    'straps_split3_bf16': (_I, [_P, _P, _L, _L, _P]),
    'straps_split3_bf16_cm': (_I, [_P, _P, _L, _I, _L, _P]),
    'straps_conv_fwd_x3': (_I, [_P, _L, _P, _L, _P, _P, _P, _I, _P, _P, _I, _I, _I, _I, _I, _I, _I, _I, _I, _I, _P]),
    'straps_conv_fwd_x3p': (_I, [_P, _L, _P, _L, _P, _P, _P, _I, _P, _P, _L, _I, _I, _I, _I, _I, _I, _I, _I, _I, _I, _P]),
    'straps_conv_dgrad_x3': (_I, [_P, _L, _P, _L, _P, _P, _I, _I, _I, _I, _I, _I, _I, _I, _I, _I, _P]),
    'straps_split_bf16_cm': (_I, [_P, _P, _L, _I, _P]),
    'straps_pack_conv_weight_bf16': (_I, [_P, _P, _I, _I, _I, _I, _P]),
    'straps_conv_bf16_tile_choice': (_I, [_I] * 9),
    'straps_conv_fwd_bf16': (_I, [_P, _P, _P, _P, _P, _I, _P, _P] + [_I] * 10 + [_P]),
    'straps_conv_x3_stat_blocks': (_I, [_I] * 10),
    'straps_conv_x3f_supported': (_I, [_I] * 6),
    'straps_conv_fwd_x3f': (_I, [_P, _P, _P, _I, _P, _L, _P, _P, _P, _I, _P, _P] + [_I] * 10 + [_P]),
    'straps_conv_x3f_stat_blocks': (_I, [_I] * 10),
    'straps_conv_dgrad_x3f': (_I, [_P, _P, _L, _P, _P, _P] + [_I] * 10 + [_P] * 8),
    'straps_conv_dgrad_x3f_bn_blocks': (_I, [_I] * 10),
    'straps_conv_wgrad_x3f_workspace_bytes': (_Z, [_I] * 9),
    'straps_conv_wgrad_x3f': (_I, [_P, _P, _P, _I, _P, _P, _P] + [_I] * 10 + [_P]),
    'straps_bn_apply_x3': (_I, [_P, _P, _P, _P, _I, _P, _P, _L, _L, _I, _P]),
    'straps_bn_relu_maxpool_fwd_x3': (_I, [_P, _P, _P, _P, _P, _P, _L, _I, _I, _I, _I, _P]),
    'straps_conv_wgrad_x3_on_planes': (_I, [_I] * 9),
    'straps_conv_dgrad_x3_bn_blocks': (_I, [_I] * 10),
    'straps_conv_dgrad_x3_bn': (_I, [_P, _L, _P, _L, _P, _P, _I, _I, _I, _I, _I, _I, _I, _I, _I, _I, _P, _P, _P, _P, _P, _P, _P, _P]),
    'straps_bn_bwd_finish_x3': (_I, [_P] * 13 + [_L, _P, _I, _P, _L, _I, _I, _P]),
    'straps_conv_wgrad_x3': (_I, [_P, _P, _P, _L, _P, _L, _P, _P, _I, _I, _I, _I, _I, _I, _I, _I, _I, _I, _P]),
    'straps_bn_bwd_x3': (_I, [_P] * 13 + [_L, _P, _L, _I, _I, _P]),
    'straps_bn_apply_bits_x3': (_I, [_P, _P, _P, _P, _P, _P, _L, _P, _L, _I, _P]),
    'straps_bn_bwd_bits_x3': (_I, [_P] * 10 + [_L, _P, _L, _I, _I, _P]),
    'straps_bn_bwd_finish_bits_x3': (_I, [_P] * 10 + [_L, _P, _I, _P, _L, _I, _I, _P]),
    'straps_conv_dgrad_x3_bits': (_I, [_P, _L, _P, _L, _P, _P, _I, _I, _I, _I, _I, _I, _I, _I, _I, _I, _P, _P]),
    'straps_conv_dgrad_x3_bn_bits': (_I, [_P, _L, _P, _L, _P, _P, _I, _I, _I, _I, _I, _I, _I, _I, _I, _I, _P, _P, _P, _P, _P, _P, _P, _P, _P, _P]),
    'straps_conv_stat_blocks': (_I, [_I, _I, _I, _I, _I, _I]),
    'straps_conv_fwd': (_I, [_P, _P, _P, _P, _P, _I, _P, _P, _I, _I, _I, _I, _I, _I, _I, _I, _I, _I, _P]),
    'straps_maxpool_fwd': (_I, [_P, _P, _I, _I, _I, _I, _P]),
    'straps_gap_fwd': (_I, [_P, _P, _I, _I, _I, _P]),
    'straps_bn_stats_finalize': (_I, [_P, _I, _I, _L, _P, _P, _F, _F, _P, _P, _P, _P, _P, _P, _P]),
    'straps_bn_apply': (_I, [_P, _P, _P, _P, _I, _P, _L, _I, _P]),
    'straps_linear_fwd': (_I, [_P, _I, _P, _I, _P, _P, _P, _I, _I, _I, _I, _I, _P]),
    'straps_broadcast_rows': (_I, [_P, _I, _P, _I, _I, _P]),
    'straps_ief_pack': (_I, [_P, _P, _P, _P, _P, _I, _I, _I, _I, _I, _P]),
    'straps_gemm_multi': (_I, [C.POINTER(GemmDesc), _I, _P]),
    'straps_rot6d_fwd': (_I, [_P, _L, _I, _P, _L, _P]),
    'straps_rodrigues_fwd': (_I, [_P, _P, _L, _P]),
    'straps_rodrigues_bwd': (_I, [_P, _P, _P, _L, _P]),
    'straps_orthographic_project': (_I, [_P, _P, _I, _P, _L, _I, _P]),
    'straps_orthographic_project_bwd': (_I, [_P, _P, _I, _P, _P, _P, _L, _I, _P]),
    'straps_perspective_project': (_I, [_P, _P, _P, _P, _I, _P, _L, _I, _P]),
    'straps_smpl_workspace_bytes': (_Z, [C.POINTER(SmplModelStruct), _L]),
    'straps_smpl_fwd': (_I, [C.POINTER(SmplModelStruct), _P, _P, _P, _P, _P, _L, _I, _I, _P]),
    'straps_smpl_bwd_workspace_bytes': (_Z, [_L, _I]),
    'straps_smpl_bwd': (_I, [C.POINTER(SmplModelStruct), _P, _P, _P, _P, _P, _P, _P, _L, _I, _P]),
    'straps_smpl_bwd_aa': (_I, [C.POINTER(SmplModelStruct), _P, _P, _P, _P, _P, _P, _P, _P, _P, _L, _I, _P]),
    'straps_conv_dgrad': (_I, [_P, _P, _P, _P, _I, _I, _I, _I, _I, _I, _I, _I, _I, _I, _P]),
    'straps_conv_wgrad_workspace_bytes': (_Z, [_I, _I, _I, _I, _I, _I, _I, _I, _I]),
    'straps_conv_wgrad': (_I, [_P, _P, _P, _P, _I, _I, _I, _I, _I, _I, _I, _I, _I, _I, _P]),
    'straps_conv_wgrad_plan': (_I, [_I] * 10 + [C.POINTER(WgradPlanStruct)]),
    'straps_stem_wgrad_workspace_bytes': (_Z, [_I, _I, _I, _I]),
    'straps_stem_wgrad': (_I, [_P, _P, _P, _P, _P, _I, _I, _I, _I, _I, _P]),
    'straps_stem_dgrad_weight_floats': (_Z, [_I]),
    'straps_pack_stem_dgrad_weight': (_I, [_P, _P, _I, _P]),
    'straps_stem_dgrad': (_I, [_P, _P, _P, _I, _I, _I, _I, _I, _P]),
    'straps_bn_bwd_blocks': (_I, [_L, _I]),
    'straps_bn_bwd_workspace_bytes': (_Z, [_L, _I]),
    'straps_bn_bwd': (_I, [_P, _P, _P, _P, _P, _P, _P, _P, _P, _P, _P, _P, _P, _L, _I, _I, _P]),
    'straps_bn_relu_maxpool_fwd': (_I, [_P, _P, _P, _P, _P, _I, _I, _I, _I, _P]),
    'straps_bn_bwd_pooled': (_I, [_P, _P, _P, _P, _P, _P, _P, _P, _P, _P, _P, _P, _I, _I, _I, _I, _I, _P]),
    'straps_bn_bwd_pooled_sparse': (_I, [_P, _P, _P, _P, _P, _P, _P, _P, _P, _P, _P, _P, _I, _I, _I, _I, _I, _P, _P]),
    'straps_stem_tiles': (_Z, [_I, _I, _I]),
    'straps_stem_tile_activity': (_I, [_P, _P, _I, _I, _I, _I, _P]),
    'straps_maxpool_fwd_idx': (_I, [_P, _P, _P, _I, _I, _I, _I, _P]),
    'straps_maxpool_bwd': (_I, [_P, _P, _P, _I, _I, _I, _I, _P]),
    'straps_gap_bwd': (_I, [_P, _P, _I, _I, _I, _P]),
    'straps_masked_copy': (_I, [_P, _I, _P, _I, _P, _I, _I, _I, _I, _P]),
    'straps_rot6d_bwd': (_I, [_P, _L, _I, _P, _P, _L, _L, _P]),
    'straps_build_proxy_input': (_I, [_P, _P, _P, _I, _I, _I, _P]),
    'straps_build_proxy_input_std': (_I, [_P, _P, _P, _I, _I, _I, _I, _P]),
    'straps_build_proxy_input_nz': (_I, [_P, _P, _P, _P, _I, _I, _I, _I, _P]),
    'straps_loss_workspace_bytes': (_Z, [_L]),
    'straps_loss_fwd_bwd': (_I, [_P, _P, _P, _I, _P, _P, _P, _P, _P, _P, _P, _P, _P, _P, _P, _P, _P, _P, _L, _I, _P]),
    'straps_loss_fwd_bwd_gm': (_I, [_P, _P, _P, _I, _P, _P, _P, _P, _P, _P, _P, _P, _P, _P, _P, _P, _P, _P, _L, _I, _P, _F, _P]),
    'straps_count_visible': (_I, [_P, _P, _L, _I, _I, _P]),
    'straps_adam_step': (_I, [_P, _P, _P, _P, _L, _I, _F, _F, _F, _F, _F, _P, _P]),
    'straps_mse_fwd': (_I, [_P, _P, _P, _L, _I, _F, _F, _P, _P, _P]),
    'straps_mse_bwd': (_I, [_P, _P, _P, _L, _I, _F, _F, _P, _P, _P]),
    'straps_augment_seg': (_I, [_P, _P, _P, _F, _I, _P, _I, _I, _P]),
    'straps_rasterize_workspace_bytes': (_Z, [_L, _I, _I]),
    'straps_rasterize_parts': (_I, [_P, _P, _P, _P, _P, _P, _P, _P, _P, _L, _I, _I, _I, _I, _F, _F, _P, _D, _D, _P]),
    'straps_philox_fill': (_I, [C.c_ulonglong, _P, _L, C.c_uint, _P, _L, _I, _P]),
    'straps_counter_add': (_I, [_P, _I, _L, _P]),
    'straps_gather_f32': (_I, [_P, _P, _P, _I, _P]),
    'straps_memset_zero': (_I, [_P, _Z, _P]),
    'straps_augment_smpl': (_I, [_P, _L, _P, _P, _P, _P, _I, _P, _D, _D, _P, _P, _P, _L, _P]),
    'straps_augment_cam_t': (_I, [_P, _P, _P, _D, _D, _D, _P, _L, _P]),
    'straps_deviate_verts2d': (_I, [_P, _P, _D, _D, _P, _L, _P]),
    'straps_deviate_joints2d': (_I, [_P, _P, _D, _D, _D, _D, _P, _L, _P]),
    'straps_project_targets': (_I, [_P, _P, _F, _F, _F, _F, _P, _P, _L, _P]),
    'straps_point_metrics': (_I, [_P, _P, _P, _L, _I, _P]),
    'straps_crop_resize': (_I, [_P, _P, _P, _D, _D, _D, _D, _D, _P, _P, _P, _I, _I, _I, _I, _P]),
    'straps_predict_proxy_input': (_I, [_P, _P, _I, _P, _I, _D, _P, _P, _P, _I, _I, _I, _I, _I, _P]),
    'straps_point_align': (_I, [_P, _P, _P, _P, _P, _L, _I, _P]),
    'straps_silhouette_counts': (_I, [_P, _P, _P, _L, _L, _P]),
    'straps_wp_silhouette_workspace_bytes': (_Z, [_L, _I]),
    'straps_wp_silhouette': (_I, [_P, _P, _P, _P, _P, _L, _I, _I, _I, _P]),
    'straps_fit_keypoints': (_I, [C.POINTER(FitModelStruct), C.POINTER(FitOptsStruct)] + [_P] * 11 + [_L, _P]),
    'straps_distance_field': (_I, [_P, _P, _L, _I, _P]),
    'straps_silhouette_energy_workspace_bytes': (_Z, [_L, _I, _I, _I]),
    'straps_silhouette_energy': (_I, [_P, _P, _I, _P, _P, C.POINTER(SilFitOptsStruct)] + [_P] * 5 + [_L, _I, _P]),
    'straps_fit_adam': (_I, [C.POINTER(FitOptsStruct)] + [_P] * 7 + [_F, _F] + [_P] * 3 + [_L, _L] + [_P] * 3 + [_I, _I, _I, _L, _P]),
    'straps_render_mesh_workspace_bytes': (_Z, [_L, _I, _I]),
    'straps_render_mesh': (_I, [_P, _P, _P, _P, _P, _I, _P, _I, C.POINTER(RenderOptsStruct)] + [_P] * 6 + [_L, _I, _I, _I, _P]),
    'straps_measure_workspace_bytes': (_Z, [_L, _I, _I, _I]),
    'straps_measure_mesh': (_I, [_P, _P, _P, _P, C.POINTER(MeasureStruct), _P, _P, _L, _I, _I, _I, _I, _P]),
    'straps_comm_unique_id': (_I, [_P]),
    'straps_comm_init_rank': (_I, [_P, _I, _I, C.POINTER(C.c_void_p)]),
    'straps_comm_destroy': (_I, [_P]),
    'straps_comm_size': (_I, [_P]),
    'straps_comm_library': (C.c_char_p, []),
    'straps_allreduce_grads': (_I, [_P, _L, _P, _P]),
    'straps_regressor_param_floats': (_Z, [C.POINTER(RegressorDesc)]),
    'straps_regressor_prepared_bytes': (_Z, [C.POINTER(RegressorDesc)]),
    'straps_regressor_prepare': (_I, [C.POINTER(RegressorDesc), _P, _P, _P]),
    'straps_regressor_workspace_bytes': (_Z, [C.POINTER(RegressorDesc), _I, _I, _I]),
    'straps_regressor_fwd_infer': (_I, [C.POINTER(RegressorDesc), _P, _P, _I, _I, _I, _P, _I, _P, _P, _Z, _P]),
    'straps_regressor_train_param_floats': (_Z, [C.POINTER(RegressorDesc)]),
    'straps_regressor_bn_state_floats': (_Z, [C.POINTER(RegressorDesc)]),
    'straps_regressor_train_workspace_bytes': (_Z, [C.POINTER(RegressorDesc), _I, _I, _I]),
    'straps_regressor_fwd_train': (_I, [C.POINTER(RegressorDesc), _P, _P, _P, _P, _I, _I, _I, _P, _I, _P, _Z, _P]),
    'straps_regressor_bwd': (_I, [C.POINTER(RegressorDesc), _P, _P, _I, _I, _I, _P, _I, _P, _P, _P, _Z, _P]),
    'straps_regressor_export_infer_params': (_I, [C.POINTER(RegressorDesc), _P, _P, _P, _P, _P]),
}


def load(path=None):
    global _lib
    if _lib is not None and path is None:
        return _lib
    p = path or LIB_PATH
    if not os.path.isfile(p):
        raise RuntimeError('libstraps_hip.so is not built (%s missing): run `python -c "import __graft_entry__ as g; '
                           'g.build()"` -- this package has no CPU fallback' % p)
    if os.path.abspath(p) != os.path.abspath(TOOLS_LIB_PATH):
        _audit(p, 'hipabi.load')
    lib = C.CDLL(p)
    if hasattr(lib, 'straps_abi_version'):
        lib.straps_abi_version.restype = C.c_int
        got = lib.straps_abi_version()
        if got != ABI_VERSION:
            raise RuntimeError('%s is ABI version %d, this package binds version %d: rebuild it (`python -c "import __graft_entry__ as g; g.build()"`)'
                               % (p, got, ABI_VERSION))
    for name, (res, args) in SIGNATURES.items():
# ... 88 lines not shown
```

straps-3dhumanshapepose_amd/train_step.py:

```python
import ctypes as C
import sys

import numpy as np
import torch

from . import config, hipabi
from .autograd_ops import encoder_backward, ief_backward
from .encoder_exec import encoder_forward
from .ief_module import EST_LD
from .multi_task_loss import TASKS

SMPL_AUGMENT_PARAMS = {'augment_shape': True, 'delta_betas_distribution': 'normal', 'delta_betas_std_vector': [1.5] * 10,
                       'delta_betas_range': [-3., 3.]}
CAM_AUGMENT_PARAMS = {'xy_std': 0.05, 'delta_z_range': [-5, 5]}
BBOX_AUGMENT_PARAMS = {'crop_input': True, 'mean_scale_factor': 1.2, 'delta_scale_range': [-0.2, 0.2], 'delta_centre_range': [-5, 5]}
PROXY_REP_AUGMENT_PARAMS = {'remove_appendages': True, 'deviate_joints2D': True, 'deviate_verts2D': True, 'occlude_seg': True,
                            'remove_appendages_classes': [1, 2, 3, 4, 5, 6],
                            'remove_appendages_probabilities': [0.1, 0.1, 0.1, 0.1, 0.05, 0.05],
                            'delta_j2d_dev_range': [-8, 8], 'delta_j2d_hip_dev_range': [-8, 8], 'delta_verts2d_dev_range': [-0.01, 0.01],
                            'occlude_probability': 0.5, 'occlude_box_dim': 48}
H36M14 = [73 + i for i in config.H36M_TO_J14]


def flatten_parameters(params, device):
# ... 159 lines not shown
        self.comm_overlap = bool(comm_overlap)
        split_off, off = 0, 0
        for n_, p_ in regressor.named_parameters():
            if n_.startswith('image_encoder.layer3.'):
                split_off = off
                break
            off += p_.numel()
        self.tail_offset = split_off
        self.exchange = GradientExchange(self.flat_g, split_off if self.comm_overlap else 0, world_size, group, force=self._force_exchange,
                                         backend=self._exchange_backend, rank=rank)
        self.time_exchange, self.exchange_events = False, []
        self.logvar_params = [getattr(criterion, n + '_log_var') for n in TASKS]
        self._lv_index = None
        if all(p.requires_grad and p in self.gviews for p in self.logvar_params):
            offs = [(self.gviews[p].data_ptr() - self.flat_g.data_ptr()) // 4 for p in self.logvar_params]
            base = min(offs)
            if sorted(o - base for o in offs) == list(range(5)):
                rel = [o - base for o in offs]
                inv = [rel.index(i) for i in range(5)]
                self._lv_index = torch.tensor(rel, dtype=torch.int32, device=self.dev)
                self._lv_index_inv = torch.tensor(inv, dtype=torch.int32, device=self.dev)
                self._lv_params_flat = self.flat_p[base:base + 5]
                self._lv_grads_flat = self.flat_g[base:base + 5]
        from .device_rng import DeviceDraws
        self.draws = DeviceDraws(seed + rank, self.dev)
        self.smpl_augment_params = dict(SMPL_AUGMENT_PARAMS if smpl_augment_params is None else smpl_augment_params)
        self.cam_augment_params = dict(CAM_AUGMENT_PARAMS if cam_augment_params is None else cam_augment_params)
        self.bbox_augment_params = dict(BBOX_AUGMENT_PARAMS if bbox_augment_params is None else bbox_augment_params)
        self.proxy_rep_augment_params = dict(PROXY_REP_AUGMENT_PARAMS if proxy_rep_augment_params is None else proxy_rep_augment_params)
        assert self.smpl_augment_params['delta_betas_distribution'] in ['uniform', 'normal']
        self.step_t = torch.zeros(1, dtype=torch.int64, device=self.dev)
        self.use_graph, self.graph, self.graph_tail, self._warm, self._g_loss = use_graph, None, None, 0, None
        self.side_stream = torch.cuda.Stream(device=self.dev) if overlap_wgrad else None
        d = self.dev
        self.mean_shape = torch.zeros(10, device=d) if mean_shape is None else torch.as_tensor(mean_shape, dtype=torch.float32, device=d)
        self.mean_cam_t = torch.tensor(mean_cam_t, device=d).expand(batch_size, 3).contiguous()
        self._eye = torch.eye(3, device=d).expand(batch_size, 24, 3, 3).contiguous()
        K = np.array([[config.FOCAL_LENGTH, 0., config.REGRESSOR_IMG_WH / 2.0], [0., config.FOCAL_LENGTH, config.REGRESSOR_IMG_WH / 2.0],
                      [0., 0., 1.]], dtype=np.float32)
        self.cam_K = torch.from_numpy(K).to(d)
        from .augmentation import remove_probabilities
        self.remove_prob = remove_probabilities(self.proxy_rep_augment_params, d)
        std = self.smpl_augment_params.get('delta_betas_std_vector')
        self._std_vector = None if std is None else torch.as_tensor(std, dtype=torch.float32, device=d).expand(10).contiguous()
        self.pool_shape = self.mean_shape[None].expand(batch_size, 10).contiguous()
        if renderer is None:
            if smpl.faces is None or smpl.face_parts is None:
                raise RuntimeError('TrainStep: the SMPL model carries no faces / face_parts; pass renderer=NMRRenderer(...)')
            from .nmr_renderer import NMRRenderer
            renderer = NMRRenderer(batch_size, self.cam_K.cpu(), torch.eye(3), config.REGRESSOR_IMG_WH, rend_parts_seg=True,
                                   faces=smpl.faces, face_parts=smpl.face_parts).to(d)
        self.renderer = renderer
        self.metrics = None
        if track_metrics:
            from .metrics import BatchMetrics
            self.metrics = BatchMetrics(self.dev)
        self._coco = torch.tensor(config.ALL_JOINTS_TO_COCO_MAP, device=d)
        self._h36m14 = torch.tensor([config.ALL_JOINTS_TO_H36M_MAP[k] for k in config.H36M_TO_J14], device=d)
        bns = [m for m in regressor.image_encoder.modules() if isinstance(m, torch.nn.BatchNorm2d) and m.track_running_stats
               and m.num_batches_tracked is not None]
        self.nbt_flat = torch.stack([m.num_batches_tracked.detach().to(d) for m in bns]) if bns else None
        for k, m in enumerate(bns):
            m.num_batches_tracked = self.nbt_flat[k]
        regressor.image_encoder._nbt_flat = self.nbt_flat
        if pose_pool is None:
            g = torch.Generator().manual_seed(seed)
            pose_pool = torch.randn(4096, 72, generator=g) * 0.2
            pose_pool[:, :3] = 0
            pose_pool[:, 1] = (torch.rand(4096, generator=g) * 2 - 1) * np.pi * 0.5
        self.pose_pool = pose_pool.to(d)
        self.last = {}
        self.pipeline = bool(pipeline_data)
        self.data_stream = torch.cuda.Stream(device=d) if self.pipeline else None
        self._bufs = [self._new_buffers() for _ in range(2)] if self.pipeline else None
        self._cur, self._primed = 0, False
        self._last_by_parity = {}

    def _new_buffers(self):
        d, B = self.dev, self.B
        return dict(input=torch.empty(B, 18, 256, 256, device=d), verts=torch.empty(B, 6890, 3, device=d),
                    joints2d=torch.empty(B, 17, 2, device=d), joints3d=torch.empty(B, 14, 3, device=d),
                    shape=torch.empty(B, 10, device=d), rot=torch.empty(B, 24, 3, 3, device=d),
                    reposed=torch.empty(B, 6890, 3, device=d), cam_t=torch.empty(B, 3, device=d), vis_count=torch.zeros(1, device=d),
                    nzmask=torch.empty(hipabi.lib().straps_stem_nzmask_words(B, 18, 256, 256), device=d, dtype=torch.int32))

    def draw_layout(self):
        B = self.B
        u, off = {}, 0
        for name, n in (('pose_index', B), ('cam_z', B), ('crop', 3 * B), ('seg', 9 * B), ('joints2d', 34 * B), ('shape_uniform', 10 * B),
                        ('verts2d', 2 * 6890 * B)):
            u[name] = (off, n)
            off += (n + 3) // 4 * 4
        n_shape = (10 * B + 3) // 4 * 4
        return {'uniform': u, 'n_uniform': off, 'normal': {'shape': (0, 10 * B), 'cam_xy': (n_shape, 2 * B)}, 'n_normal': n_shape + 2 * B}

    def make_batch(self, out=None, keep=None):
        L, st, d, B = hipabi.lib(), hipabi.stream_ptr(), self.dev, self.B
        out = self._new_buffers() if out is None else out
        lay = self.draw_layout()
        U = self.draws.fill(torch.empty(lay['n_uniform'], device=d), 0, 0)
        N = self.draws.fill(torch.empty(lay['n_normal'], device=d), 1, 1)
        self.draws.advance()

        def useg(name):
            o, n = lay['uniform'][name]
            return U[o:o + n]

        def nseg(name):
            o, n = lay['normal'][name]
            return N[o:o + n]
        sp, cp, bp, pp = self.smpl_augment_params, self.cam_augment_params, self.bbox_augment_params, self.proxy_rep_augment_params
        mode = 0
        if sp['augment_shape']:
            mode = 1 if sp['delta_betas_distribution'] == 'normal' else 2
        sdraws = nseg('shape') if mode == 1 else useg('shape_uniform')
        rng = sp['delta_betas_range'] if mode == 2 else (0.0, 0.0)
        tgt_shape, tgt_rot = out['shape'], out['rot']
        hipabi.check(L.straps_augment_smpl(hipabi.ptr(self.pose_pool), self.pose_pool.shape[0], hipabi.ptr(useg('pose_index')),
                                           hipabi.ptr(self.pool_shape), hipabi.ptr(self.mean_shape), hipabi.ptr(sdraws), mode, hipabi.ptr(self._std_vector),
                                           float(rng[0]), float(rng[1]), hipabi.ptr(tgt_shape), hipabi.ptr(tgt_rot), None, B, st),
                     'straps_augment_smpl')
        cam_t = out['cam_t']
        hipabi.check(L.straps_augment_cam_t(hipabi.ptr(self.mean_cam_t), hipabi.ptr(nseg('cam_xy')), hipabi.ptr(useg('cam_z')), float(cp['xy_std']),
                                            float(cp['delta_z_range'][0]), float(cp['delta_z_range'][1]), hipabi.ptr(cam_t), B, st),
                     'straps_augment_cam_t')
        tgt_verts, tgt_joints = self.smpl.forward_arrays(tgt_shape, tgt_rot, out_verts=out['verts'])
        self.smpl.forward_arrays(tgt_shape, self._eye, want_joints=False, out_verts=out['reposed'])
        j2d_full = torch.empty(B, 17, 2, device=d)
        wh = float(config.REGRESSOR_IMG_WH)
        hipabi.check(L.straps_project_targets(hipabi.ptr(tgt_joints), hipabi.ptr(cam_t), config.FOCAL_LENGTH, config.FOCAL_LENGTH, wh / 2, wh / 2,
                                              hipabi.ptr(j2d_full), hipabi.ptr(out['joints3d']), B, st), 'straps_project_targets')
        noise = useg('verts2d') if pp['deviate_verts2D'] else None
        seg = self.renderer.render_arrays(tgt_verts, cam_t, vert_noise_u=noise, noise_range=pp['delta_verts2d_dev_range'])
        if bp['crop_input']:
            from .image_utils import batch_crop_and_resize
            seg_c, tgt_j2d, boxes = batch_crop_and_resize(seg, j2d_full, config.REGRESSOR_IMG_WH, bp['mean_scale_factor'], bp['delta_scale_range'],
                                                          bp['delta_centre_range'], uniforms=useg('crop'), jout=out['joints2d'])
        else:
            seg_c, boxes = seg, None
            tgt_j2d = out['joints2d']
            hipabi.check(L.straps_masked_copy(hipabi.ptr(j2d_full), 34, None, 0, hipabi.ptr(tgt_j2d), 34, B, 34, 0, st), 'joints2d copy')
        seg_aug = torch.empty_like(seg_c)
        hipabi.check(L.straps_augment_seg(hipabi.ptr(seg_c), hipabi.ptr(useg('seg')), hipabi.ptr(self.remove_prob),
                                          float(pp['occlude_probability']) if pp['occlude_seg'] else 0.0, int(pp['occlude_box_dim']),
                                          hipabi.ptr(seg_aug), B, 256, st), 'straps_augment_seg')
        j2d_in = tgt_j2d
        if pp['deviate_joints2D']:
            j2d_in = torch.empty(B, 17, 2, device=d)
            r, hr = pp['delta_j2d_dev_range'], pp['delta_j2d_hip_dev_range']
            hipabi.check(L.straps_deviate_joints2d(hipabi.ptr(tgt_j2d), hipabi.ptr(useg('joints2d')), float(r[0]), float(r[1]), float(hr[0]),
                                                   float(hr[1]), hipabi.ptr(j2d_in), B, st), 'straps_deviate_joints2d')
        x = out['input']
        if _FUSED_PROXY_NZ:
            hipabi.check(L.straps_build_proxy_input_nz(hipabi.ptr(seg_aug), hipabi.ptr(j2d_in), hipabi.ptr(x), hipabi.ptr(out['nzmask']), B, 17, 256, 4, st),
                         'straps_build_proxy_input_nz')
        else:
            hipabi.check(L.straps_build_proxy_input(hipabi.ptr(seg_aug), hipabi.ptr(j2d_in), hipabi.ptr(x), B, 17, 256, st), 'straps_build_proxy_input')
            hipabi.check(L.straps_stem_nzmask(hipabi.ptr(x), hipabi.ptr(out['nzmask']), B, 18, 256, 256, st), 'straps_stem_nzmask')
        hipabi.check(L.straps_count_visible(hipabi.ptr(tgt_j2d), hipabi.ptr(out['vis_count']), B, 17, config.REGRESSOR_IMG_WH, st), 'straps_count_visible')
        if keep is not None:
            keep.update(uniforms=U, normals=N, joints=tgt_joints, joints2d_uncropped=j2d_full, seg=seg, seg_cropped=seg_c, boxes=boxes,
                        seg_aug=seg_aug, joints2d_input=j2d_in)
        return out

    def forward_backward(self, batch, after_layer3=None):
        L, st, d, B = hipabi.lib(), hipabi.stream_ptr(), self.dev, self.B
        reg, smpl = self.reg, self.smpl
        assert reg.training, 'TrainStep needs the regressor in .train() mode'
        hipabi.check(L.straps_memset_zero(hipabi.ptr(self.flat_g), self.flat_g.numel() * 4, st), 'straps_memset_zero(flat gradient)')
        enc_tape, ief_tape = {}, []
        reg.image_encoder.prepack(with_dgrad=True)
        if self.nbt_flat is not None:
            hipabi.check(L.straps_counter_add(hipabi.ptr(self.nbt_flat), self.nbt_flat.numel(), 1, st), 'straps_counter_add(num_batches_tracked)')
        feat = encoder_forward(reg.image_encoder, batch['input'], enc_tape, nzmask=batch.get('nzmask'))
        est = reg.ief_module.forward_estimate(feat, ief_tape)
        pose6d = est[:, 3:147]
        R = torch.empty(B, 24, 3, 3, device=d)
        hipabi.check(L.straps_rot6d_fwd(hipabi.ptr(pose6d), EST_LD, 24, hipabi.ptr(R), B, st), 'straps_rot6d_fwd')
        pred_shape = torch.empty(B, 10, device=d)
        hipabi.check(L.straps_masked_copy(C.c_void_p(est.data_ptr() + 4 * 147), EST_LD, None, 0, hipabi.ptr(pred_shape), 10, B, 10, 0, st), 'pred_shape')
        verts, joints = smpl.forward_arrays(pred_shape, R)
        eye = self._eye
        reposed, _ = smpl.forward_arrays(pred_shape, eye, want_joints=False)
        if self._lv_index is not None:
            lv = torch.empty(5, device=d)
            hipabi.check(L.straps_gather_f32(hipabi.ptr(self._lv_params_flat), hipabi.ptr(self._lv_index), hipabi.ptr(lv), 5, st), 'log-var gather')
        else:
            lv = self.crit.log_var_vector()
        loss = torch.empty(12, device=d)
        dverts, djoints = torch.empty_like(verts), torch.empty_like(joints)
        dest, drot = torch.empty(B, EST_LD, device=d), torch.empty(B, 24, 3, 3, device=d)
        dlv = torch.empty(5, device=d)
        ws = torch.empty(L.straps_loss_workspace_bytes(B) // 4, device=d)
        gm = getattr(self, 'global_masked_mean', False)
        hipabi.check(L.straps_loss_fwd_bwd_gm(hipabi.ptr(verts), hipabi.ptr(joints), hipabi.ptr(est), EST_LD, hipabi.ptr(R), hipabi.ptr(batch['verts']),
                                              hipabi.ptr(batch['joints2d']), hipabi.ptr(batch['joints3d']), hipabi.ptr(batch['shape']),
                                              hipabi.ptr(batch['rot']), hipabi.ptr(lv), hipabi.ptr(loss), hipabi.ptr(dverts), hipabi.ptr(djoints),
                                              hipabi.ptr(dest), hipabi.ptr(drot), hipabi.ptr(dlv), hipabi.ptr(ws), B, config.REGRESSOR_IMG_WH,
                                              hipabi.ptr(batch['vis_count'] if gm else None), 1.0 / self.world, st),
                     'straps_loss_fwd_bwd')
        dbetas, drot2 = torch.empty(B, 10, device=d), torch.empty(B, 24, 3, 3, device=d)
        ws2 = torch.empty(L.straps_smpl_bwd_workspace_bytes(B, 0) // 4, device=d)
        hipabi.check(L.straps_smpl_bwd(C.byref(smpl._model_struct()), hipabi.ptr(pred_shape), hipabi.ptr(R), hipabi.ptr(dverts), hipabi.ptr(djoints),
                                       hipabi.ptr(dbetas), hipabi.ptr(drot2), hipabi.ptr(ws2), B, 0, st), 'straps_smpl_bwd')
        hipabi.check(L.straps_masked_copy(hipabi.ptr(drot2), 216, None, 0, hipabi.ptr(drot), 216, B, 216, 1, st), 'drot sum')
        hipabi.check(L.straps_masked_copy(hipabi.ptr(dbetas), 10, None, 0, C.c_void_p(dest.data_ptr() + 4 * 147), EST_LD, B, 10, 1, st), 'dshape sum')
        hipabi.check(L.straps_rot6d_bwd(hipabi.ptr(pose6d), EST_LD, 24, hipabi.ptr(drot), C.c_void_p(dest.data_ptr() + 4 * 3), EST_LD, B, st),
                     'straps_rot6d_bwd')
        dfeat, _ = ief_backward(reg.ief_module, feat, ief_tape, dest, self.gviews)
        if self._lv_index is not None:
            hipabi.check(L.straps_gather_f32(hipabi.ptr(dlv), hipabi.ptr(self._lv_index_inv), hipabi.ptr(self._lv_grads_flat), 5, st), 'log-var gradient scatter')
        else:
            for k, p in enumerate(self.logvar_params):
                if p.requires_grad:
                    self.gviews[p].copy_(dlv[k])
        encoder_backward(reg.image_encoder, enc_tape, dfeat, self.gviews, self.side_stream, after_layer3)
        self.last = dict(loss=loss, verts=verts, joints=joints, est=est, reposed=reposed, rot=R, ief_tape=ief_tape,
                         enc_tape=enc_tape if getattr(self, 'keep_enc_tape', False) else None,
                         bwd=dict(dverts=dverts, djoints=djoints, dlv=dlv, dbetas=dbetas, drot_smpl=drot2, dest=dest, dfeat=dfeat)
                         if getattr(self, 'keep_bwd', False) else None)
        if self.metrics is not None:
            from .cam_utils import orthographic_project_torch
            pred = {'verts': verts, 'joints3D': joints.index_select(1, self._h36m14), 'shape_params': pred_shape,
                    'pose_params_rot_matrices': R,
                    'joints2D': orthographic_project_torch(joints.index_select(1, self._coco), est[:, :3])}
            tgt = {'verts': batch['verts'], 'joints3D': batch['joints3d'], 'shape_params': batch['shape'],
                   'pose_params_rot_matrices': batch['rot'], 'joints2D': batch['joints2d']}
            self.metrics.update(pred, tgt, pred_reposed_vertices=reposed, target_reposed_vertices=batch['reposed'])
        return loss

    def metrics_summary(self):
        if self.metrics is None:
            raise RuntimeError('TrainStep was built with track_metrics=False')
        self.metrics.n = self.steps * self.B
        return self.metrics.summary()

    def optimise(self):
        if self.time_exchange and self.exchange.active:
            e0, e1 = torch.cuda.Event(enable_timing=True), torch.cuda.Event(enable_timing=True)
            e0.record()
            gscale = self.exchange.finish()
            e1.record()
            self.exchange_events.append((e0, e1))
        else:
            gscale = self.exchange.finish()
        self.steps += 1
        hipabi.check(hipabi.lib().straps_counter_add(hipabi.ptr(self.step_t), 1, 1, hipabi.stream_ptr()), 'straps_counter_add(adam step)')
        hipabi.check(hipabi.lib().straps_adam_step(hipabi.ptr(self.flat_p), hipabi.ptr(self.flat_g), hipabi.ptr(self.exp_avg),
                                                   hipabi.ptr(self.exp_avg_sq), self.flat_p.numel(), self.steps, self.lr, 0.9, 0.999, 1e-8,
                                                   gscale, hipabi.ptr(self.step_t), hipabi.stream_ptr()), 'straps_adam_step')
        self.reg.image_encoder._cache.clear()
        self.reg.ief_module._cache = {}

    def _run(self, after_layer3):
        if not self.pipeline:
            b = self.make_batch()
            if self.global_masked_mean:
# ... 208 lines not shown
```

Baseline: 8079.

## Skip inactive stem tiles in fused BN-ReLU-maxpool forward and pooled BN backward

Computes the stem tile-activity map once, during batch construction, and carries it through the encoder tape so forward and backward both reuse it. The fused BN+ReLU+maxpool forward becomes a tiled kernel that stages a BN-applied patch in shared memory and skips loads for inactive map tiles through buffer-load masking. The pooled BN backward moves to a per-tile kernel that exits early on inactive tiles and routes pooled gradients in registers. Gains depend on input sparsity, and the new tile indexing raises correctness risk at borders.

```diff
diff --git a/include/straps_hip.h b/include/straps_hip.h
--- a/include/straps_hip.h
+++ b/include/straps_hip.h
@@ -327,6 +327,13 @@
                                 const float* mask_scale, const float* mask_shift, float* dgamma,
                                 float* dbeta, float* draw, void* workspace, int batch, int h, int w, int c,
                                 int accumulate, const uint8_t* tile_active, void* stream);
+int straps_bn_relu_maxpool_fwd_sparse(const float* raw_nhwc, const float* scale, const float* shift,
+                                      float* y_pool_nhwc, uint8_t* idx, int batch, int h, int w, int c,
+                                      const uint8_t* tile_active, void* stream);
+int straps_bn_relu_maxpool_fwd_x3_sparse(const float* raw, const float* scale, const float* shift,
+                                         float* y_pool, uint8_t* idx, unsigned short* y_planes,
+                                         long long plane_stride, int batch, int h, int w, int c,
+                                         const uint8_t* tile_active, void* stream);
 int straps_maxpool_fwd_idx(const float* x_nhwc, float* y_nhwc, uint8_t* idx, int batch, int h,
                            int w, int c, void* stream);
 int straps_maxpool_bwd(const float* dy_nhwc, const uint8_t* idx, float* dx_nhwc, int batch, int h,
diff --git a/straps-3dhumanshapepose_amd/autograd_ops.py b/straps-3dhumanshapepose_amd/autograd_ops.py
--- a/straps-3dhumanshapepose_amd/autograd_ops.py
+++ b/straps-3dhumanshapepose_amd/autograd_ops.py
@@ -262,12 +262,7 @@
         ws = torch.empty(L.straps_bn_bwd_workspace_bytes(B * H * W, Cc) // 4, device=raw.device, dtype=torch.float32)
         dgamma, dbeta = grads.buf(bn.weight), grads.buf(bn.bias)
         draw = _empty_like(raw)
-        tact = None
-        if rec.get('nzmask') is not None and _SPARSE_STEM_TAIL and not want_dx:
-            _, Cin0, Hin, Win = rec['geom'][:4]
-            tact = torch.empty(L.straps_stem_tiles(B, Hin, Win), device=raw.device, dtype=torch.uint8)
-            hipabi.check(L.straps_stem_tile_activity(hipabi.ptr(rec['nzmask']), hipabi.ptr(tact), B, Cin0, Hin, Win, hipabi.stream_ptr()),
-                         'straps_stem_tile_activity')
+        tact = rec.get('tile_active') if _SPARSE_STEM_TAIL and not want_dx else None
         hipabi.check(L.straps_bn_bwd_pooled_sparse(hipabi.ptr(dy), hipabi.ptr(idx), hipabi.ptr(raw), hipabi.ptr(ss[2]), hipabi.ptr(ss[3]),
                                                    hipabi.ptr(bn.weight), hipabi.ptr(ss[0]), hipabi.ptr(ss[1]), hipabi.ptr(dgamma), hipabi.ptr(dbeta),
                                                    hipabi.ptr(draw), hipabi.ptr(ws), B, H, W, Cc, 2 if rec.get('frozen') else 0, hipabi.ptr(tact),
diff --git a/straps-3dhumanshapepose_amd/csrc/backward.hip b/straps-3dhumanshapepose_amd/csrc/backward.hip
--- a/straps-3dhumanshapepose_amd/csrc/backward.hip
+++ b/straps-3dhumanshapepose_amd/csrc/backward.hip
@@ -449,19 +449,15 @@
     }
 }
 
-constexpr int POOL_CHUNK = 1024;
-template <bool POOL>
 __global__ __launch_bounds__(256) void bn_bwd_apply_kernel(const float* __restrict__ dy, const float* __restrict__ yact,
                                                            const float* __restrict__ raw, const float* __restrict__ mean,
                                                            const float* __restrict__ invstd, const double* __restrict__ coefd,
                                                            const float* __restrict__ k1p, const float* __restrict__ msc,
                                                            const float* __restrict__ msh, float* __restrict__ draw, float* dz_out,
-                                                           u16* __restrict__ planes, long long pstride, long long n4, int C, PoolSrc ps,
+                                                           u16* __restrict__ planes, long long pstride, long long n4, int C,
                                                            const unsigned* __restrict__ bits, int tiled) {
     const int C4 = C >> 2;
-    const long long first = POOL ? (long long)blockIdx.x * POOL_CHUNK + threadIdx.x : (long long)blockIdx.x * 256 + threadIdx.x;
-    const long long last = POOL ? (n4 < ((long long)blockIdx.x + 1) * POOL_CHUNK ? n4 : ((long long)blockIdx.x + 1) * POOL_CHUNK) : n4;
-    const long long step = POOL ? 256 : (long long)gridDim.x * 256;
+    const long long first = (long long)blockIdx.x * 256 + threadIdx.x, last = n4, step = (long long)gridDim.x * 256;
     const long long rows = n4 / C4;
     struct Consts { f32x4 ksc, ksh, mu, is, k1; double m1[4], m2[4]; };
     auto load_consts = [&](int c4) {
@@ -475,19 +471,7 @@
         return k;
     };
     auto body = [&](long long idx, long long row, int c4, const Consts& k) {
-        f32x4 g;
-        if constexpr (POOL) {
-            if (ps.tany) {
-                const int wi = (int)(row % ps.W);
-                const long long t = row / ps.W;
-                const int hi = (int)(t % ps.H);
-                const long long b = t / ps.H;
-                if (!ps.tany[(b * ps.tiles_y + (hi >> 1)) * ps.tiles_x + (wi >> 5)]) return;
-            }
-            g = pool_grad(ps, row, c4, C);
-        } else {
-            g = *reinterpret_cast<const f32x4*>(dy + idx * 4);
-        }
+        f32x4 g = *reinterpret_cast<const f32x4*>(dy + idx * 4);
         const f32x4 xr = *reinterpret_cast<const f32x4*>(raw + idx * 4);
         if (bits) {
             const unsigned nib = bits[row * (C >> 5) + (c4 >> 3)] >> ((c4 & 7) * 4);
@@ -511,7 +495,7 @@
         if (draw) *reinterpret_cast<f32x4*>(draw + idx * 4) = o;
         if (planes) store_planes4_cm(planes, pstride, row, c4 * 4, rows, o);
     };
-    if (!POOL && tiled) {
+    if (tiled) {
         const int l = threadIdx.x & 63, w = threadIdx.x >> 6, wcg = tiled, ncb = (C4 >> 4) / wcg, trows = 16 / wcg;
         const int c4 = ((int)(blockIdx.x % ncb) * wcg + w % wcg) * 16 + (l >> 5) * 8 + (l & 7);
         const Consts k = load_consts(c4);
@@ -532,6 +516,85 @@
     }
 }
 
+typedef unsigned u32x4 __attribute__((ext_vector_type(4)));
+__global__ __launch_bounds__(256) __attribute__((amdgpu_waves_per_eu(4))) void bn_bwd_apply_pool_tile_kernel(const float* __restrict__ raw, const float* __restrict__ mean,
+                                                                     const float* __restrict__ invstd, const double* coefd,
+                                                                     const float* __restrict__ k1p, const float* __restrict__ msc,
+                                                                     const float* __restrict__ msh, float* __restrict__ draw, int C, PoolSrc ps) {
+    static_assert(TY == 2 && TX == 32, "two columns per thread, both tile rows");
+    if (ps.tany && !ps.tany[blockIdx.x]) return;
+    const int cl = threadIdx.x & 15, pl = threadIdx.x >> 4;
+    const bool chan = (blockIdx.y * 16 + cl) * 4 < C;
+    const int c4 = chan ? blockIdx.y * 16 + cl : 0;
+    int tile = blockIdx.x;
+    const int per_image = ps.tiles_x * ps.tiles_y, b = __builtin_amdgcn_readfirstlane(tile / per_image);
+    tile -= b * per_image;
+    const int ty = __builtin_amdgcn_readfirstlane(tile / ps.tiles_x), tx = tile - ty * ps.tiles_x;
+    const int h0 = ty * TY, w0 = tx * TX;
+    const int row1 = h0 + 1 < ps.H ? 1 : 0;
+    const int dh = ty + 1 < ps.Ho ? 1 : 0;
+    const long long tbase = (((long long)b * ps.H + h0) * ps.W + w0) * C, pbase = ((long long)b * ps.Ho + ty) * ps.Wo * C;
+    const float* rawt = raw + tbase + c4 * 4;
+    const float* dyt = ps.dyp + pbase + c4 * 4;
+    const uint8_t* idt = ps.idx + pbase + c4 * 4;
+    const __amdgpu_buffer_rsrc_t rs_draw = __builtin_amdgcn_make_buffer_rsrc(draw + tbase, 0, __builtin_amdgcn_readfirstlane(((row1 + 1) * ps.W - w0) * C * 4), 0x00020000);
+    f32x4 xr[2][2], d[2][4];
+    unsigned k[2][4];
+    int roff[2], odd[2];
+    bool inside[2], ok_hi[2];
+#pragma unroll
+    for (int q = 0; q < 2; ++q) {
+        const int col = q * 16 + pl, colc = w0 + col < ps.W ? col : ps.W - 1 - w0;
+        inside[q] = colc == col;
+        roff[q] = colc * C;
+        const int wi = w0 + colc, wlo = wi >> 1, whi = (wi + 1) >> 1 < ps.Wo ? (wi + 1) >> 1 : ps.Wo - 1;
+        odd[q] = wi & 1;
+        ok_hi[q] = odd[q] && (wi + 1) >> 1 < ps.Wo;
+#pragma unroll
+        for (int j = 0; j < 4; ++j) {
+            const int o = ((j >> 1) * dh * ps.Wo + ((j & 1) ? whi : wlo)) * C;
+            k[q][j] = *reinterpret_cast<const unsigned*>(idt + o);
+            d[q][j] = *reinterpret_cast<const f32x4*>(dyt + o);
+        }
+        xr[q][0] = *reinterpret_cast<const f32x4*>(rawt + roff[q]);
+        xr[q][1] = *reinterpret_cast<const f32x4*>(rawt + row1 * ps.W * C + roff[q]);
+    }
+    const f32x4 ksc = *reinterpret_cast<const f32x4*>(msc + c4 * 4), ksh = *reinterpret_cast<const f32x4*>(msh + c4 * 4);
+    const f32x4 mu = *reinterpret_cast<const f32x4*>(mean + c4 * 4), is = *reinterpret_cast<const f32x4*>(invstd + c4 * 4);
+    const f32x4 k1 = *reinterpret_cast<const f32x4*>(k1p + c4 * 4);
+    double m1[4], m2[4];
+#pragma unroll
+    for (int e = 0; e < 4; ++e) { m1[e] = coefd[c4 * 4 + e]; m2[e] = coefd[C + c4 * 4 + e]; }
+    __builtin_amdgcn_sched_barrier(0);
+#pragma unroll
+    for (int q = 0; q < 2; ++q) {
+#pragma unroll
+        for (int j = 0; j < 4; ++j) asm volatile("" : "+v"(k[q][j]), "+v"(d[q][j]));
+        asm volatile("" : "+v"(xr[q][0]), "+v"(xr[q][1]));
+#pragma unroll
+        for (int row = 0; row < 2; ++row) {
+            f32x4 g = {0.f, 0.f, 0.f, 0.f};
+#pragma unroll
+            for (int j = 0; j < (row ? 4 : 2); ++j) {
+                const int want = (row ? ((j >> 1) ? 0 : 2) : 1) * 3 + ((j & 1) ? 0 : odd[q] + 1);
+                const bool ok = ((j & 1) ? ok_hi[q] : true) & ((j >> 1) ? dh != 0 : true);
+#pragma unroll
+                for (int e = 0; e < 4; ++e)
+                    if (ok & ((int)((k[q][j] >> (8 * e)) & 0xffu) == want)) g[e] += d[q][j][e];
+            }
+            f32x4 o;
+#pragma unroll
+            for (int e = 0; e < 4; ++e) {
+                g[e] = fmaf(xr[q][row][e], ksc[e], ksh[e]) > 0.f ? g[e] : 0.f;
+                const double xh = ((double)xr[q][row][e] - (double)mu[e]) * (double)is[e];
+                o[e] = (float)((double)k1[e] * (((double)g[e] - m1[e]) - xh * m2[e]));
+            }
+            const bool st = inside[q] & (row <= row1) & chan;
+            __builtin_amdgcn_raw_buffer_store_b128(__builtin_bit_cast(u32x4, o), rs_draw, (unsigned)(row * ps.W * C + roff[q] + c4 * 4) * 4u | ((unsigned)st - 1u), 0, 0);
+        }
+    }
+}
+
 __global__ __launch_bounds__(256) void maxpool_idx_kernel(const float* __restrict__ x, float* __restrict__ y, uint8_t* __restrict__ idx,
                                                           int B, int H, int W, int C, int Ho, int Wo) {
     const int C4 = C >> 2;
@@ -565,42 +628,92 @@
     }
 }
 
-__global__ __launch_bounds__(256) void bn_relu_maxpool_kernel(const float* __restrict__ raw, const float* __restrict__ scale,
-                                                              const float* __restrict__ shift, float* __restrict__ y, uint8_t* __restrict__ idx,
-                                                              u16* __restrict__ planes, long long pstride, int B, int H, int W, int C, int Ho, int Wo) {
-    const int C4 = C >> 2;
-    const long long n = (long long)B * Ho * Wo * C4;
-    for (long long i = (long long)blockIdx.x * 256 + threadIdx.x; i < n; i += (long long)gridDim.x * 256) {
-        const int c4 = (int)(i % C4);
-        long long t = i / C4;
-        const int wo = (int)(t % Wo); t /= Wo;
-        const int ho = (int)(t % Ho);
-        const int b = (int)(t / Ho);
-        const f32x4 sc = *reinterpret_cast<const f32x4*>(scale + c4 * 4);
-        const f32x4 sh = *reinterpret_cast<const f32x4*>(shift + c4 * 4);
+constexpr int FT_PY = 2, FT_PX = 16, FT_RH = 2 * FT_PY + 1, FT_RW = 2 * FT_PX + 1, FT_N = FT_RH * FT_RW, FT_TRIPS = (FT_N + 15) / 16;
+static_assert(TY == 2 && 2 * FT_PX == TX, "the patch lies under map tiles (ho0 - 1 .. ho0 + FT_PY - 1) x (px - 1, px): pooled row ho <-> map row ho");
+__global__ __launch_bounds__(256) void bn_relu_maxpool_tile_kernel(const float* __restrict__ raw, const float* __restrict__ scale,
+                                                                   const float* __restrict__ shift, float* __restrict__ y, uint8_t* __restrict__ idx,
+                                                                   u16* __restrict__ planes, long long pstride, int B, int H, int W, int C, int Ho, int Wo,
+                                                                   const uint8_t* __restrict__ tany, int tiles_x, int tiles_y, int ptx, int pty) {
+    __shared__ f32x4 patch[FT_TRIPS * 16][16];
+    const int cl = threadIdx.x & 15, pl = threadIdx.x >> 4;
+    const int c4 = blockIdx.y * 16 + cl;
+    const bool chan = c4 * 4 < C;
+    int t = blockIdx.x;
+    const int per_image = ptx * pty, b = __builtin_amdgcn_readfirstlane(t / per_image);
+    t -= b * per_image;
+    const int py = __builtin_amdgcn_readfirstlane(t / ptx), px = t - py * ptx;
+    const int ho0 = py * FT_PY, wo0 = px * FT_PX;
+    const int hi0 = 2 * ho0 - 1, wi0 = 2 * wo0 - 1;
+    const int hb = hi0 < 0 ? 0 : hi0;
+    const int nrows = H - hb < FT_RH ? H - hb : FT_RH;
+    const __amdgpu_buffer_rsrc_t rs = __builtin_amdgcn_make_buffer_rsrc(const_cast<float*>(raw) + ((long long)b * H + hb) * W * C, 0, nrows * W * C * 4, 0x00020000);
+    unsigned mbits = 0x3fu;
+    if (tany) {
+        unsigned char mv[6];
+#pragma unroll
+        for (int q = 0; q < 6; ++q) {
+            const int my = ho0 - 1 + (q >> 1), mx = px - 1 + (q & 1);
+            const int myc = my < 0 ? 0 : (my < tiles_y ? my : tiles_y - 1), mxc = mx < 0 ? 0 : (mx < tiles_x ? mx : tiles_x - 1);
+            mv[q] = tany[((long long)b * tiles_y + myc) * tiles_x + mxc];
+        }
+        mbits = 0;
+#pragma unroll
+        for (int q = 0; q < 6; ++q) {
+            const int my = ho0 - 1 + (q >> 1), mx = px - 1 + (q & 1);
+            mbits |= (unsigned)((my >= 0) & (my < tiles_y) & (mx >= 0) & (mx < tiles_x) & (mv[q] != 0)) << q;
+        }
+    }
+    const int cs = chan ? c4 : 0;
+    const f32x4 sc = *reinterpret_cast<const f32x4*>(scale + cs * 4);
+    const f32x4 sh = *reinterpret_cast<const f32x4*>(shift + cs * 4);
+    u32x4 x[FT_TRIPS];
+#pragma unroll
+    for (int j = 0; j < FT_TRIPS; ++j) {
+        const int p = pl + 16 * j, rr = p / FT_RW, cc = p - rr * FT_RW;
+        const int hi = hi0 + rr, wi = wi0 + cc;
+        const unsigned wanted = (unsigned)chan & (unsigned)(p < FT_N) & (unsigned)((unsigned)hi < (unsigned)H) & (unsigned)((unsigned)wi < (unsigned)W) & (mbits >> (((rr + 1) >> 1) * 2 + (cc > 0)));
+        const unsigned off = (unsigned)(((hi - hb) * W + wi) * C + c4 * 4) * 4u | ((wanted & 1u) - 1u);
+        x[j] = __builtin_amdgcn_raw_buffer_load_b128(rs, off, 0, 0);
+    }
+    __builtin_amdgcn_sched_barrier(0);
+#pragma unroll
+    for (int j = 0; j < FT_TRIPS; ++j) {
+        const int p = pl + 16 * j;
+        f32x4 v;
+#pragma unroll
+        for (int e = 0; e < 4; ++e) v[e] = fmaxf(fmaf(__uint_as_float(x[j][e]), sc[e], sh[e]), 0.f);
+        patch[p][cl] = v;
+    }
+    __syncthreads();
+    if (!chan || wo0 + pl >= Wo) return;
+    const int wo = wo0 + pl;
+#pragma unroll
+    for (int dy = 0; dy < FT_PY; ++dy) {
+        const int ho = ho0 + dy;
+        if (ho >= Ho) break;
         f32x4 m = {-INFINITY, -INFINITY, -INFINITY, -INFINITY};
         int am[4] = {0, 0, 0, 0};
         bool first = true;
 #pragma unroll
         for (int r = 0; r < 3; ++r) {
-            const int hi = 2 * ho - 1 + r;
-            if ((unsigned)hi >= (unsigned)H) continue;
 #pragma unroll
             for (int s = 0; s < 3; ++s) {
-                const int wi = 2 * wo - 1 + s;
-                if ((unsigned)wi >= (unsigned)W) continue;
-                f32x4 v = *reinterpret_cast<const f32x4*>(raw + (((long long)b * H + hi) * W + wi) * C + c4 * 4);
-#pragma unroll
-                for (int e = 0; e < 4; ++e) {
-                    v[e] = fmaxf(fmaf(v[e], sc[e], sh[e]), 0.f);
-                    if (first || v[e] > m[e] || v[e] != v[e]) { m[e] = v[e]; am[e] = r * 3 + s; }
+                const bool inb = (unsigned)(2 * ho - 1 + r) < (unsigned)H && (unsigned)(2 * wo - 1 + s) < (unsigned)W;
+                const f32x4 v = patch[(2 * dy + r) * FT_RW + 2 * pl + s][cl];
+#pragma unroll
+                for (int e = 0; e < 4; ++e)
+                {
+                    const bool take = inb & (first | (v[e] > m[e]) | (v[e] != v[e]));
+                    m[e] = take ? v[e] : m[e];
+                    am[e] = take ? r * 3 + s : am[e];
                 }
-                first = false;
-            }
-        }
-        *reinterpret_cast<f32x4*>(y + i * 4) = m;
-        *reinterpret_cast<uchar4*>(idx + i * 4) = make_uchar4((unsigned char)am[0], (unsigned char)am[1], (unsigned char)am[2], (unsigned char)am[3]);
-        if (planes) store_planes4_cm(planes, pstride, i / C4, c4 * 4, (long long)B * Ho * Wo, m);
+                first = first & !inb;
+            }
+        }
+        const long long row = ((long long)b * Ho + ho) * Wo + wo;
+        *reinterpret_cast<f32x4*>(y + row * C + c4 * 4) = m;
+        *reinterpret_cast<uchar4*>(idx + row * C + c4 * 4) = make_uchar4((unsigned char)am[0], (unsigned char)am[1], (unsigned char)am[2], (unsigned char)am[3]);
+        if (planes) store_planes4_cm(planes, pstride, row, c4 * 4, (long long)B * Ho * Wo, m);
     }
 }
 
@@ -798,7 +911,7 @@
     STRAPS_CHECK_LAUNCH("bn_bwd_finalize_kernel");
     const long long n4 = rows * C4;
     const int tiled = straps_bn_tiled(rows, c >> 2);
-    hipLaunchKernelGGL(bn_bwd_apply_kernel<false>, dim3(tiled ? straps_bn_tiled_grid(rows, c >> 2, tiled) : straps_grid256_rows(n4, c >> 2)), dim3(256), 0, st, dy, yact, raw, save_mean, save_invstd, coefd, k1, mask_scale, mask_shift, draw, dz_out, draw_planes, plane_stride, n4, c, PoolSrc{}, relu_bits, tiled);
+    hipLaunchKernelGGL(bn_bwd_apply_kernel, dim3(tiled ? straps_bn_tiled_grid(rows, c >> 2, tiled) : straps_grid256_rows(n4, c >> 2)), dim3(256), 0, st, dy, yact, raw, save_mean, save_invstd, coefd, k1, mask_scale, mask_shift, draw, dz_out, draw_planes, plane_stride, n4, c, relu_bits, tiled);
     STRAPS_CHECK_LAUNCH("bn_bwd_apply_kernel");
     return STRAPS_OK;
 }
@@ -838,7 +951,7 @@
     STRAPS_CHECK_LAUNCH("bn_bwd_finalize_kernel");
     const long long n4 = rows * C4;
     const int tiled = straps_bn_tiled(rows, c >> 2);
-    hipLaunchKernelGGL(bn_bwd_apply_kernel<false>, dim3(tiled ? straps_bn_tiled_grid(rows, c >> 2, tiled) : straps_grid256_rows(n4, c >> 2)), dim3(256), 0, st, dy, yact, raw, save_mean, save_invstd, coefd, k1, mask_scale, mask_shift, draw, dz_out, draw_planes, plane_stride, n4, c, PoolSrc{}, relu_bits, tiled);
+    hipLaunchKernelGGL(bn_bwd_apply_kernel, dim3(tiled ? straps_bn_tiled_grid(rows, c >> 2, tiled) : straps_grid256_rows(n4, c >> 2)), dim3(256), 0, st, dy, yact, raw, save_mean, save_invstd, coefd, k1, mask_scale, mask_shift, draw, dz_out, draw_planes, plane_stride, n4, c, relu_bits, tiled);
     STRAPS_CHECK_LAUNCH("bn_bwd_apply_kernel");
     return STRAPS_OK;
 }
@@ -915,27 +1028,41 @@
     STRAPS_CHECK_LAUNCH("bn_bwd_reduce_pooled_kernel");
     hipLaunchKernelGGL(bn_bwd_finalize_kernel, dim3((c + 3) / 4), dim3(256), 0, st, part, nblk, c, bn_bwd_count(rows, accumulate), gamma, save_invstd, dgamma, dbeta, coefd, k1, accumulate & 1);
     STRAPS_CHECK_LAUNCH("bn_bwd_finalize_kernel");
-    const long long n4 = rows * C4;
-    hipLaunchKernelGGL(bn_bwd_apply_kernel<true>, dim3((unsigned)((n4 + POOL_CHUNK - 1) / POOL_CHUNK)), dim3(256), 0, st, nullptr, nullptr, raw, save_mean, save_invstd, coefd, k1, mask_scale, mask_shift, draw, nullptr, (u16*)nullptr, 0LL, n4, c, ps, (const unsigned*)nullptr, 0);
-    STRAPS_CHECK_LAUNCH("bn_bwd_apply_kernel<pool>");
+    STRAPS_REQUIRE((long long)w * c < (1LL << 27) && (long long)batch * ps.tiles_x * ps.tiles_y < (1LL << 31), "straps_bn_bwd_pooled: row of %d x %d floats or batch %d too large for the tile walk", w, c, batch);
+    hipLaunchKernelGGL(bn_bwd_apply_pool_tile_kernel, dim3((unsigned)(batch * ps.tiles_x * ps.tiles_y), (c + 63) / 64), dim3(256), 0, st, raw, save_mean, save_invstd, coefd, k1, mask_scale, mask_shift, draw, c, ps);
+    STRAPS_CHECK_LAUNCH("bn_bwd_apply_pool_tile_kernel");
     return STRAPS_OK;
 }
 
 extern "C" int straps_bn_relu_maxpool_fwd_x3(const float* raw, const float* scale, const float* shift, float* y_pool, uint8_t* idx,
                                              unsigned short* y_planes, long long plane_stride, int batch, int h, int w, int c, void* stream) {
+    return straps_bn_relu_maxpool_fwd_x3_sparse(raw, scale, shift, y_pool, idx, y_planes, plane_stride, batch, h, w, c, nullptr, stream);
+}
+
+extern "C" int straps_bn_relu_maxpool_fwd_x3_sparse(const float* raw, const float* scale, const float* shift, float* y_pool, uint8_t* idx,
+                                                    unsigned short* y_planes, long long plane_stride, int batch, int h, int w, int c,
+                                                    const uint8_t* tile_active, void* stream) {
     STRAPS_REQUIRE(raw && scale && shift && y_pool && idx && batch > 0 && h > 0 && w > 0 && c > 0 && (c & 3) == 0, "straps_bn_relu_maxpool_fwd: bad arguments");
     const int Ho = (h - 1) / 2 + 1, Wo = (w - 1) / 2 + 1;
     const long long n = (long long)batch * Ho * Wo * (c >> 2);
     STRAPS_REQUIRE(!y_planes || (plane_stride >= n * 4 && plane_stride % 8 == 0), "straps_bn_relu_maxpool_fwd_x3: plane_stride must be >= the output size and a multiple of 8");
     STRAPS_REQUIRE(!y_planes || (c & 31) == 0, "straps_bn_relu_maxpool_fwd_x3: chunk-major planes need c %% 32 == 0 (c=%d)", c);
-    hipLaunchKernelGGL(bn_relu_maxpool_kernel, dim3(capped_grid(n)), dim3(256), 0, (hipStream_t)stream, raw, scale, shift, y_pool, idx, y_planes, plane_stride, batch, h, w, c, Ho, Wo);
-    STRAPS_CHECK_LAUNCH("bn_relu_maxpool_kernel");
+    const int ptx = (Wo + FT_PX - 1) / FT_PX, pty = (Ho + FT_PY - 1) / FT_PY;
+    STRAPS_REQUIRE((long long)w * c < (1LL << 26) && (long long)batch * ptx * pty < (1LL << 31), "straps_bn_relu_maxpool_fwd: row of %d x %d floats or batch %d too large for the tile walk", w, c, batch);
+    hipLaunchKernelGGL(bn_relu_maxpool_tile_kernel, dim3((unsigned)(batch * ptx * pty), (c + 63) / 64), dim3(256), 0, (hipStream_t)stream, raw, scale, shift, y_pool, idx, y_planes, plane_stride, batch, h, w, c, Ho, Wo,
+                       tile_active, (w + TX - 1) / TX, (h + TY - 1) / TY, ptx, pty);
+    STRAPS_CHECK_LAUNCH("bn_relu_maxpool_tile_kernel");
     return STRAPS_OK;
 }
 
 extern "C" int straps_bn_relu_maxpool_fwd(const float* raw, const float* scale, const float* shift, float* y_pool, uint8_t* idx, int batch, int h,
                                           int w, int c, void* stream) {
-    return straps_bn_relu_maxpool_fwd_x3(raw, scale, shift, y_pool, idx, nullptr, 0, batch, h, w, c, stream);
+    return straps_bn_relu_maxpool_fwd_x3_sparse(raw, scale, shift, y_pool, idx, nullptr, 0, batch, h, w, c, nullptr, stream);
+}
+
+extern "C" int straps_bn_relu_maxpool_fwd_sparse(const float* raw, const float* scale, const float* shift, float* y_pool, uint8_t* idx, int batch, int h,
+                                                 int w, int c, const uint8_t* tile_active, void* stream) {
+    return straps_bn_relu_maxpool_fwd_x3_sparse(raw, scale, shift, y_pool, idx, nullptr, 0, batch, h, w, c, tile_active, stream);
 }
 
 extern "C" size_t straps_bn_bwd_workspace_bytes(long long rows, int c) {
diff --git a/straps-3dhumanshapepose_amd/csrc/regressor_train.hip b/straps-3dhumanshapepose_amd/csrc/regressor_train.hip
--- a/straps-3dhumanshapepose_amd/csrc/regressor_train.hip
+++ b/straps-3dhumanshapepose_amd/csrc/regressor_train.hip
@@ -297,11 +297,13 @@
     RG_CALL(straps_stem_nzmask(x, nz, B, C, h, w, stream));
     RG_CALL(straps_stem_fwd(x, ws.f(p.wstem), nullptr, nullptr, 0, ws.f(p.stem_raw), part, nz, B, C, h, w, stream));
     RG_CALL(finalize(params, bn_state, part, p.stem_nblk, 64, (long long)B * p.geo.Hs * p.geo.Ws, p.stem.gb_off, p.stem.rs_off, sss, st));
+    uint8_t* tact = (uint8_t*)(ws.base + p.tact);
+    RG_CALL(straps_stem_tile_activity(nz, tact, B, C, h, w, stream));
     if (p.pool_planes)
-        RG_CALL(straps_bn_relu_maxpool_fwd_x3(ws.f(p.stem_raw), sss, sss + 64, ws.f(p.pool), (uint8_t*)(ws.base + p.idx), ws.h(p.pool3), p.pool_ps,
-                                              B, p.geo.Hs, p.geo.Ws, 64, stream));
+        RG_CALL(straps_bn_relu_maxpool_fwd_x3_sparse(ws.f(p.stem_raw), sss, sss + 64, ws.f(p.pool), (uint8_t*)(ws.base + p.idx), ws.h(p.pool3), p.pool_ps,
+                                                     B, p.geo.Hs, p.geo.Ws, 64, tact, stream));
     else
-        RG_CALL(straps_bn_relu_maxpool_fwd(ws.f(p.stem_raw), sss, sss + 64, ws.f(p.pool), (uint8_t*)(ws.base + p.idx), B, p.geo.Hs, p.geo.Ws, 64, stream));
+        RG_CALL(straps_bn_relu_maxpool_fwd_sparse(ws.f(p.stem_raw), sss, sss + 64, ws.f(p.pool), (uint8_t*)(ws.base + p.idx), B, p.geo.Hs, p.geo.Ws, 64, tact, stream));
 
     auto conv_fwd = [&](const Layer& cv) -> int {
         const float* sa = cv.a_bn ? ws.f(cv.a_bn->ss) : nullptr;
@@ -552,11 +554,7 @@
 
     const float* sss = ws.f(p.stem_ss);
     const uint32_t* nz = (const uint32_t*)(ws.base + p.nz);
-    uint8_t* tact = nullptr;
-    if (!dx) {
-        tact = (uint8_t*)(ws.base + p.tact);
-        RG_CALL(straps_stem_tile_activity(nz, tact, B, C, h, w, stream));
-    }
+    const uint8_t* tact = dx ? nullptr : (const uint8_t*)(ws.base + p.tact);
     float* sdraw = ws.f(p.sdraw);
     RG_CALL(straps_bn_bwd_pooled_sparse(ws.f(p.g[cur]), (const uint8_t*)(ws.base + p.idx), ws.f(p.stem_raw), sss + 128, sss + 192, params + p.stem.gb_off,
                                         sss, sss + 64, dgamma(p.stem.gb_off), dbeta(p.stem.gb_off, 64), sdraw, bnws, B, p.geo.Hs, p.geo.Ws, 64, 0, tact, stream));
diff --git a/straps-3dhumanshapepose_amd/encoder_exec.py b/straps-3dhumanshapepose_amd/encoder_exec.py
--- a/straps-3dhumanshapepose_amd/encoder_exec.py
+++ b/straps-3dhumanshapepose_amd/encoder_exec.py
@@ -232,7 +232,7 @@
     return out, Ho, Wo
 
 
-def encoder_forward(net, x, tape=None, nzmask=None):
+def encoder_forward(net, x, tape=None, nzmask=None, tile_active=None):
     hipabi.require_gpu_tensor(x, 'encoder input', torch.float32)
     if x.dim() != 4 or x.shape[1] != net.in_channels:
         raise RuntimeError('encoder expects [B,%d,H,W], got %s' % (net.in_channels, tuple(x.shape)))
@@ -268,6 +268,16 @@
         hipabi.check(L.straps_stem_nzmask(hipabi.ptr(x), hipabi.ptr(nzmask), B, C, H, W, hipabi.stream_ptr()), 'straps_stem_nzmask')
     if rec is not None:
         rec['nzmask'] = nzmask
+        ntiles = L.straps_stem_tiles(B, H, W)
+        if getattr(net, 'unfused_stem_tail', False):
+            tile_active = None
+        elif tile_active is not None and not getattr(net, 'dense_stem', False):
+            if tile_active.dtype != torch.uint8 or tile_active.numel() != ntiles or tile_active.device != x.device or not tile_active.is_contiguous():
+                raise RuntimeError('encoder_forward: tile_active must be a contiguous uint8 tensor of %d entries on %s' % (ntiles, x.device))
+        else:
+            tile_active = torch.empty(ntiles, device=x.device, dtype=torch.uint8)
+            hipabi.check(L.straps_stem_tile_activity(hipabi.ptr(nzmask), hipabi.ptr(tile_active), B, C, H, W, hipabi.stream_ptr()), 'straps_stem_tile_activity')
+        rec['tile_active'] = tile_active
     if not net.training and tape is None:
         ss = net._folded_bn(net.bn1)
         hipabi.check(L.straps_stem_fwd(hipabi.ptr(x), hipabi.ptr(wfrag), hipabi.ptr(ss[0]), hipabi.ptr(ss[1]), 1, hipabi.ptr(y),
@@ -287,13 +297,14 @@
             cons = [u0.conv_bn_pairs()[0][0]] + ([u0.downsample[0]] if u0.downsample is not None else [])
             if ctx.x3 and not all(x3f_mode(ctx, cv, B, Hp, Wp) for cv in cons):
                 planes, pstride = _new_planes(p)
-                hipabi.check(L.straps_bn_relu_maxpool_fwd_x3(hipabi.ptr(y), hipabi.ptr(ss[0]), hipabi.ptr(ss[1]), hipabi.ptr(p), hipabi.ptr(idx),
-                                                             hipabi.ptr(planes), pstride, B, H, W, 64, hipabi.stream_ptr()),
-                             'straps_bn_relu_maxpool_fwd_x3')
+                hipabi.check(L.straps_bn_relu_maxpool_fwd_x3_sparse(hipabi.ptr(y), hipabi.ptr(ss[0]), hipabi.ptr(ss[1]), hipabi.ptr(p), hipabi.ptr(idx),
+                                                                    hipabi.ptr(planes), pstride, B, H, W, 64, hipabi.ptr(rec['tile_active']),
+                                                                    hipabi.stream_ptr()), 'straps_bn_relu_maxpool_fwd_x3_sparse')
                 ctx.planes[id(p)] = (p, planes, pstride)
             else:
-                hipabi.check(L.straps_bn_relu_maxpool_fwd(hipabi.ptr(y), hipabi.ptr(ss[0]), hipabi.ptr(ss[1]), hipabi.ptr(p), hipabi.ptr(idx),
-                                                          B, H, W, 64, hipabi.stream_ptr()), 'straps_bn_relu_maxpool_fwd')
+                hipabi.check(L.straps_bn_relu_maxpool_fwd_sparse(hipabi.ptr(y), hipabi.ptr(ss[0]), hipabi.ptr(ss[1]), hipabi.ptr(p), hipabi.ptr(idx),
+                                                                 B, H, W, 64, hipabi.ptr(rec['tile_active']), hipabi.stream_ptr()),
+                             'straps_bn_relu_maxpool_fwd_sparse')
             tape['maxpool'] = dict(kind='maxpool_fused', out=p, idx=idx, geom=(B, H, W, 64, Hp, Wp))
             return _residual_stages(ctx, net, p, B, Hp, Wp, tape)
         y = _bn_train_finish(ctx, net.bn1, y, part, nblk, B * Ho * Wo, None, True, rec, planes=False)
diff --git a/straps-3dhumanshapepose_amd/hipabi.py b/straps-3dhumanshapepose_amd/hipabi.py
--- a/straps-3dhumanshapepose_amd/hipabi.py
+++ b/straps-3dhumanshapepose_amd/hipabi.py
@@ -245,6 +245,8 @@
     'straps_bn_relu_maxpool_fwd': (_I, [_P, _P, _P, _P, _P, _I, _I, _I, _I, _P]),
     'straps_bn_bwd_pooled': (_I, [_P, _P, _P, _P, _P, _P, _P, _P, _P, _P, _P, _P, _I, _I, _I, _I, _I, _P]),
     'straps_bn_bwd_pooled_sparse': (_I, [_P, _P, _P, _P, _P, _P, _P, _P, _P, _P, _P, _P, _I, _I, _I, _I, _I, _P, _P]),
+    'straps_bn_relu_maxpool_fwd_sparse': (_I, [_P, _P, _P, _P, _P, _I, _I, _I, _I, _P, _P]),
+    'straps_bn_relu_maxpool_fwd_x3_sparse': (_I, [_P, _P, _P, _P, _P, _P, _L, _I, _I, _I, _I, _P, _P]),
     'straps_stem_tiles': (_Z, [_I, _I, _I]),
     'straps_stem_tile_activity': (_I, [_P, _P, _I, _I, _I, _I, _P]),
     'straps_maxpool_fwd_idx': (_I, [_P, _P, _P, _I, _I, _I, _I, _P]),
diff --git a/straps-3dhumanshapepose_amd/train_step.py b/straps-3dhumanshapepose_amd/train_step.py
--- a/straps-3dhumanshapepose_amd/train_step.py
+++ b/straps-3dhumanshapepose_amd/train_step.py
@@ -265,7 +265,8 @@
                     joints2d=torch.empty(B, 17, 2, device=d), joints3d=torch.empty(B, 14, 3, device=d),
                     shape=torch.empty(B, 10, device=d), rot=torch.empty(B, 24, 3, 3, device=d),
                     reposed=torch.empty(B, 6890, 3, device=d), cam_t=torch.empty(B, 3, device=d), vis_count=torch.zeros(1, device=d),
-                    nzmask=torch.empty(hipabi.lib().straps_stem_nzmask_words(B, 18, 256, 256), device=d, dtype=torch.int32))
+                    nzmask=torch.empty(hipabi.lib().straps_stem_nzmask_words(B, 18, 256, 256), device=d, dtype=torch.int32),
+                    tile_active=torch.empty(hipabi.lib().straps_stem_tiles(B, 256, 256), device=d, dtype=torch.uint8))
 
     def draw_layout(self):
         B = self.B
@@ -340,6 +341,7 @@
         else:
             hipabi.check(L.straps_build_proxy_input(hipabi.ptr(seg_aug), hipabi.ptr(j2d_in), hipabi.ptr(x), B, 17, 256, st), 'straps_build_proxy_input')
             hipabi.check(L.straps_stem_nzmask(hipabi.ptr(x), hipabi.ptr(out['nzmask']), B, 18, 256, 256, st), 'straps_stem_nzmask')
+        hipabi.check(L.straps_stem_tile_activity(hipabi.ptr(out['nzmask']), hipabi.ptr(out['tile_active']), B, 18, 256, 256, st), 'straps_stem_tile_activity')
         hipabi.check(L.straps_count_visible(hipabi.ptr(tgt_j2d), hipabi.ptr(out['vis_count']), B, 17, config.REGRESSOR_IMG_WH, st), 'straps_count_visible')
         if keep is not None:
             keep.update(uniforms=U, normals=N, joints=tgt_joints, joints2d_uncropped=j2d_full, seg=seg, seg_cropped=seg_c, boxes=boxes,
@@ -355,7 +357,7 @@
         reg.image_encoder.prepack(with_dgrad=True)
         if self.nbt_flat is not None:
             hipabi.check(L.straps_counter_add(hipabi.ptr(self.nbt_flat), self.nbt_flat.numel(), 1, st), 'straps_counter_add(num_batches_tracked)')
-        feat = encoder_forward(reg.image_encoder, batch['input'], enc_tape, nzmask=batch.get('nzmask'))
+        feat = encoder_forward(reg.image_encoder, batch['input'], enc_tape, nzmask=batch.get('nzmask'), tile_active=batch.get('tile_active'))
         est = reg.ief_module.forward_estimate(feat, ief_tape)
         pose6d = est[:, 3:147]
         R = torch.empty(B, 24, 3, 3, device=d)
```

Result: no change. 8077 (median of 2 runs) (-0.0%).
